# jiangzhengkai/mxdetection

Hardware: AMD Instinct MI355X
Metric: images/sec (whole node) Faster R-CNN R50-FPN 3x800x1333 (higher is better)
Workload: dtype bf16; 1 GPU; Faster R-CNN ResNet-50-FPN bf16 train step, batch 2/GPU, 3x800x1333 (padded 1344); global_batch=2, parallelism=dp1, frozen=stem+C2, frozen BN folded, optimizer=SGD momentum 0.9 wd 1e-4, launch=hipGraph replay, input=resident, wgrad_side_stream=True, rpn_branch_stream=True, grouped_wgrad=True, filter_prefetch_hints=True, params_trainable=41538304

## Files before the change

include/mxdet.h:

```cpp
#ifndef MXDET_H_
#define MXDET_H_

#include <stddef.h>
#include <stdint.h>

#ifdef __cplusplus
extern "C" {
#endif

#define MXDET_OK 0
#define MXDET_EINVAL (-1)
#define MXDET_ESHAPE (-2)
#define MXDET_EWORKSPACE (-3)
#define MXDET_EHIP (-4)
#define MXDET_ERCCL (-5)

#define MXDET_DTYPE_F32 0
#define MXDET_DTYPE_BF16 1

typedef void* mxdet_stream_t;

const char* mxdet_last_error(void);
const char* mxdet_version(void);

int mxdet_box_iou(const float* boxes_a, int64_t na, const float* boxes_b, int64_t nb, float* out,
                  mxdet_stream_t stream);

int mxdet_generate_anchors(const float* base_anchors, int32_t A, int32_t H, int32_t W, int32_t stride,
                           float* out, mxdet_stream_t stream);

size_t mxdet_nms_batched_workspace_bytes(int32_t B, int32_t n_max);
int mxdet_nms_batched(const float* boxes, const int32_t* counts, const uint8_t* invalid, int32_t B,
                      int32_t n_max, float thresh, int32_t max_keep, int32_t* keep_idx,
                      int32_t* num_keep, void* workspace, size_t workspace_bytes,
                      mxdet_stream_t stream);

size_t mxdet_detection_postprocess_workspace_bytes(int32_t N, int32_t rois_per_image, int32_t num_classes);
int mxdet_detection_postprocess(const void* cls_logits, const void* bbox_pred, int32_t dtype, int32_t ld_cls,
                                int32_t ld_reg, const float* rois, const int32_t* num_rois, const float* im_info,
                                int32_t N, int32_t rois_per_image, int32_t num_classes, const float* means,
                                const float* stds, float score_thresh, float nms_thresh, int32_t max_per_image,
                                float* dets, int32_t* num_dets, void* workspace, size_t workspace_bytes,
                                mxdet_stream_t stream);


typedef struct {
  int32_t num_levels;
  int32_t A;
  int32_t H[8], W[8], stride[8];
  const void* cls[8];
  const void* reg[8];
  int64_t cls_sn[8], cls_sy[8], cls_sx[8], cls_sa[8];
  int64_t reg_sn[8], reg_sy[8], reg_sx[8], reg_sc[8];
  int32_t dtype;
  int32_t classes;
  const float* base_anchors[8];
} mxdet_pyramid_t;

size_t mxdet_proposal_workspace_bytes(const mxdet_pyramid_t* p, int32_t N, int32_t pre_nms_top_n);
int mxdet_proposal(const mxdet_pyramid_t* p, int32_t N, const float* im_info ,
                   int32_t pre_nms_top_n, int32_t post_nms_top_n, float nms_thresh, float min_size,
                   float* rois, float* roi_scores, int32_t* roi_anchor, int32_t* num_rois,
                   void* workspace, size_t workspace_bytes, mxdet_stream_t stream);

size_t mxdet_anchor_target_workspace_bytes(int32_t N, int64_t A_total, int32_t G_max);
int mxdet_anchor_target(const float* anchors, int64_t A_total, const float* gt_boxes, int32_t N,
                        int32_t G_max, const float* im_info, float fg_thresh, float bg_thresh,
                        float allowed_border, int32_t batch_size, float fg_fraction, uint32_t seed,
                        uint32_t step, const uint32_t* step_dev, uint32_t image_offset, int32_t* labels,
                        int32_t* matched_gt,
                        float* bbox_targets, float* max_iou, void* workspace, size_t workspace_bytes,
                        mxdet_stream_t stream);

int mxdet_proposal_target(const float* rois, const int32_t* num_rois, int32_t rois_stride,
                          const float* gt_boxes, int32_t N, int32_t G_max, int32_t rois_per_image,
                          float fg_fraction, float fg_thresh, float bg_hi, float bg_lo,
                          int32_t num_classes, int32_t class_agnostic,
                          const float* means , const float* stds ,
                          uint32_t seed, uint32_t step, const uint32_t* step_dev,
                          uint32_t image_offset, float* out_rois, int32_t* labels,
                          float* bbox_targets, float* bbox_weights, int32_t* matched_gt,
                          int32_t* num_fg, mxdet_stream_t stream);

int mxdet_fpn_level_map(const float* rois, int64_t R, int32_t lvl_min, int32_t lvl_max,
                        int32_t* levels, mxdet_stream_t stream);
typedef struct {
  int32_t num_levels, lvl_min;
  int32_t H[8], W[8];
  float spatial_scale[8];
  void* feat[8];
} mxdet_feat_pyramid_t;
int mxdet_roi_align_fwd(const mxdet_feat_pyramid_t* f, int32_t N, int32_t C, const float* rois,
                        const int32_t* levels, int64_t R, int32_t PH, int32_t PW,
                        int32_t sampling_ratio, uint16_t* out, mxdet_stream_t stream);
int mxdet_roi_align_bwd(const mxdet_feat_pyramid_t* f, int32_t N, int32_t C, const float* rois,
                        const int32_t* levels, int64_t R, int32_t PH, int32_t PW,
                        int32_t sampling_ratio, const uint16_t* grad_out, mxdet_stream_t stream);
size_t mxdet_roi_align_bwd_gather_workspace_bytes(const mxdet_feat_pyramid_t* f, int32_t N, int64_t R);
int mxdet_roi_align_bwd_gather(const mxdet_feat_pyramid_t* f, int32_t N, int32_t C, const float* rois,
                               const int32_t* levels, int64_t R, int32_t PH, int32_t PW, int32_t sampling_ratio,
                               const uint16_t* grad_out, int32_t accumulate, void* workspace, size_t workspace_bytes,
                               mxdet_stream_t stream);
int mxdet_roi_align_bwd_gather_prepare(const mxdet_feat_pyramid_t* f, int32_t N, const float* rois,
                                       const int32_t* levels, int64_t R, int32_t PH, int32_t PW, int32_t sampling_ratio,
                                       void* workspace, size_t workspace_bytes, mxdet_stream_t stream);
int mxdet_roi_align_bwd_gather_prepared(const mxdet_feat_pyramid_t* f, int32_t N, int32_t C, const float* rois,
                                        const int32_t* levels, int64_t R, int32_t PH, int32_t PW, int32_t sampling_ratio,
                                        const uint16_t* grad_out, int32_t accumulate, void* workspace,
                                        size_t workspace_bytes, mxdet_stream_t stream);

typedef struct {
  mxdet_feat_pyramid_t pyr;
  int32_t N, C;
  int32_t PH, PW;
  int32_t sample_per_part;
  float trans_std;
  int32_t modulated;
  int32_t trans_stride, mask_stride;
  int32_t accumulate;
} mxdet_dpool_desc_t;
int mxdet_dpool_fwd(const mxdet_dpool_desc_t* d, const float* rois, const int32_t* levels, int64_t R,
                    const uint16_t* trans, const uint16_t* mask_logit, uint16_t* out, mxdet_stream_t stream);
int mxdet_dpool_bwd_trans(const mxdet_dpool_desc_t* d, const float* rois, const int32_t* levels, int64_t R,
                          const uint16_t* trans, const uint16_t* mask_logit, const uint16_t* dout, uint16_t* d_trans,
                          uint16_t* d_mask, mxdet_stream_t stream);
size_t mxdet_dpool_bwd_feat_workspace_bytes(const mxdet_dpool_desc_t* d, int64_t R);
int mxdet_dpool_bwd_feat(const mxdet_dpool_desc_t* d, const float* rois, const int32_t* levels, int64_t R,
                         const uint16_t* trans, const uint16_t* mask_logit, const uint16_t* dout, void* workspace,
                         size_t workspace_bytes, mxdet_stream_t stream);

int mxdet_smooth_l1_fwd(const float* pred, const float* target, const float* weight, int64_t n,
                        float sigma, float* out, mxdet_stream_t stream);
int mxdet_smooth_l1_bwd(const float* pred, const float* target, const float* weight,
                        const float* grad_out, int64_t n, float sigma, int32_t accumulate,
                        float* grad_pred, mxdet_stream_t stream);

size_t mxdet_loss_workspace_bytes(int64_t n);
int mxdet_focal_loss(const void* logits, int32_t dtype, const int32_t* labels, int64_t n, int32_t C,
                     float alpha, float gamma, float grad_scale, float* loss_out, void* grad_logits,
                     void* workspace, size_t workspace_bytes, mxdet_stream_t stream);

int mxdet_anchor_class_labels(const int32_t* labels, const int32_t* matched_gt, const float* gt_boxes, int32_t N,
                              int64_t A_total, int32_t G_max, int32_t* cls_labels, int32_t* num_fg,
                              mxdet_stream_t stream);
int32_t mxdet_retina_loss_num_partials(int32_t N, int32_t H, int32_t W, int32_t A);
int mxdet_retina_loss_level(const uint16_t* cls, const uint16_t* reg, int32_t N, int32_t H, int32_t W, int32_t A,
                            int32_t C, int32_t ld_cls, int32_t ld_reg, const int32_t* cls_labels,
                            const float* bbox_targets, int64_t A_total, int64_t level_offset, float alpha,
                            float gamma, float sigma, const int32_t* num_fg, float loss_scale, uint16_t* grad_cls,
                            uint16_t* grad_reg, float* partial, mxdet_stream_t stream);

int32_t mxdet_rpn_loss_num_partials(int32_t N, int32_t H, int32_t W);
int mxdet_rpn_loss_level(const uint16_t* head, int32_t N, int32_t H, int32_t W, int32_t A,
                         int32_t Cpad, const int32_t* labels, const float* bbox_targets,
                         int64_t A_total, int64_t level_offset, float sigma, float norm,
                         float loss_scale, uint16_t* grad_head, float* partial,
                         mxdet_stream_t stream);
int mxdet_loss_finalize(const float* partial, int32_t count, int32_t ncomp, float* out,
                        mxdet_stream_t stream);

int mxdet_rcnn_loss(const void* cls_logits, const void* bbox_pred, int32_t dtype, int32_t ld_cls,
                    int32_t ld_reg, const int32_t* labels, const float* bbox_targets,
                    const float* bbox_weights, int64_t R, int32_t num_classes, int32_t reg_dim,
                    float sigma, float norm, float loss_scale, float* loss_out, void* grad_cls,
                    void* grad_reg, void* workspace, size_t workspace_bytes, mxdet_stream_t stream);

int mxdet_mask_target(const float* rois, const int32_t* matched_gt, const int32_t* labels,
                      const uint8_t* gt_masks, int64_t R, int32_t G_max, int32_t H, int32_t W, int32_t S,
                      uint8_t* targets, int32_t* cls_out, mxdet_stream_t stream);
int mxdet_pixel_shuffle2(const uint16_t* x, int64_t R, int32_t H, int32_t W, int32_t C, int32_t inverse,
                         uint16_t* y, mxdet_stream_t stream);
int mxdet_pixel_shuffle2_inv_relu(const uint16_t* dy_up, const uint16_t* act, int64_t R, int32_t H, int32_t W, int32_t C,
                                  uint16_t* dx, mxdet_stream_t stream);
size_t mxdet_mask_loss_workspace_bytes(int64_t R, int32_t S);
int mxdet_mask_loss(const uint16_t* logits, const int32_t* cls, const uint8_t* targets, int64_t R, int32_t S,
                    int32_t Cpad, float loss_scale, float* loss_out, uint16_t* grad, void* workspace,
                    size_t workspace_bytes, mxdet_stream_t stream);
size_t mxdet_mask_paste_workspace_bytes(int64_t R, int32_t S);
int mxdet_mask_paste(const uint16_t* logits, const float* dets, int64_t R, int32_t S, int32_t Cpad, int32_t H, int32_t W,
                     float thresh, uint8_t* masks, void* workspace, size_t workspace_bytes, mxdet_stream_t stream);

typedef struct {
  int32_t N, H, W, Cin;
  int32_t Cout, KH, KW;
  int32_t stride, pad;
  int32_t Ho, Wo;
  int32_t relu;
  int32_t res_upsample;
  int32_t accumulate;
  const void* prefetch;
  int64_t prefetch_bytes;
  void* relu_bits;
} mxdet_conv_desc_t;

int mxdet_conv2d_fwd(const mxdet_conv_desc_t* d, const uint16_t* x, const uint16_t* w,
                     const float* bias, const uint16_t* residual, uint16_t* y,
                     mxdet_stream_t stream);
int mxdet_conv2d_fwd_chain(const mxdet_conv_desc_t* d, const uint16_t* x, const uint16_t* w, const float* bias,
                           const uint16_t* w2, const float* bias2, int32_t cout2, int32_t relu2,
                           const uint16_t* residual2, uint16_t* y2, const uint16_t* w3, const float* bias3,
                           int32_t cout3, int32_t relu3, uint16_t* y3, mxdet_stream_t stream);
size_t mxdet_conv2d_fwd_splitk_workspace_bytes(const mxdet_conv_desc_t* d, int32_t ksplit);
int mxdet_conv2d_fwd_splitk(const mxdet_conv_desc_t* d, const uint16_t* x, const uint16_t* w, const float* bias,
                            const uint16_t* residual, uint16_t* y, int32_t ksplit, void* workspace,
                            size_t workspace_bytes, mxdet_stream_t stream);
int mxdet_conv2d_dgrad(const mxdet_conv_desc_t* d, const uint16_t* dy, const uint16_t* wt,
                       const uint16_t* residual, const uint16_t* relu_mask, uint16_t* dx,
                       mxdet_stream_t stream);
size_t mxdet_conv2d_wgrad_workspace_bytes(const mxdet_conv_desc_t* d);
int mxdet_conv2d_wgrad(const mxdet_conv_desc_t* d, const uint16_t* x, const uint16_t* dy, float* dw,
                       float* db, void* workspace, size_t workspace_bytes, mxdet_stream_t stream);
typedef struct {
  mxdet_conv_desc_t desc;
  const void* src;
  const void* filt;
  const float* bias;
  const void* residual;
  const void* relu_mask;
  void* dst;
} mxdet_conv_item_t;
size_t mxdet_conv2d_grouped_table_bytes(int32_t n);
int mxdet_conv2d_grouped_plan(const mxdet_conv_item_t* items, int32_t n, int32_t kind, void* table_host,
                              size_t table_bytes, int32_t* cfg, int32_t* grid);
int mxdet_conv2d_grouped(const void* table_dev, int32_t n, int32_t kind, int32_t cfg, int32_t grid,
                         mxdet_stream_t stream);
typedef struct {
  mxdet_conv_desc_t desc;
  const void* x;
  const void* dy;
  float* dw;
  float* db;
} mxdet_wgrad_item_t;
size_t mxdet_conv2d_wgrad_grouped_table_bytes(int32_t n);
int mxdet_conv2d_wgrad_grouped_plan(const mxdet_wgrad_item_t* items, int32_t n, void* table_host, size_t table_bytes,
                                    size_t* workspace_bytes, int32_t* grid_wgrad, int32_t* grid_big,
                                    int32_t* grid_reduce);
int mxdet_conv2d_wgrad_grouped(const void* table_dev, int32_t n, int32_t grid_wgrad, int32_t grid_big,
                               int32_t grid_reduce, void* workspace, size_t workspace_bytes, size_t workspace_needed,
                               mxdet_stream_t stream);
int mxdet_conv2d_wgrad_grouped_parts(const void* table_dev, int32_t n, int32_t grid_wgrad, int32_t grid_big,
                                     int32_t grid_reduce, int32_t parts, void* workspace, size_t workspace_bytes,
                                     size_t workspace_needed, mxdet_stream_t stream);
int mxdet_filter_transpose(const uint16_t* w, int32_t Cout, int32_t KH, int32_t KW, int32_t Cin,
                           uint16_t* wt, mxdet_stream_t stream);

int mxdet_filter_transpose_batched(const void* descs_dev, int32_t ndesc, int32_t total_tiles,
                                   mxdet_stream_t stream);

typedef struct {
  int32_t N, H, W, C;
  int32_t Ho, Wo;
  int32_t KH, KW;
  int32_t stride, pad;
  int32_t groups;
  int32_t modulated;
  int32_t off_channels;
  int32_t accumulate;
} mxdet_deform_desc_t;
int mxdet_deform_im2col(const mxdet_deform_desc_t* d, const uint16_t* x, const uint16_t* off, uint16_t* col,
                        mxdet_stream_t stream);
int mxdet_deform_col2im_coord(const mxdet_deform_desc_t* d, const uint16_t* x, const uint16_t* off,
                              const uint16_t* dcol, uint16_t* doff, mxdet_stream_t stream);
size_t mxdet_deform_col2im_workspace_bytes(const mxdet_deform_desc_t* d);
int mxdet_deform_col2im(const mxdet_deform_desc_t* d, const uint16_t* off, const uint16_t* dcol, uint16_t* dx,
                        void* workspace, size_t workspace_bytes, mxdet_stream_t stream);

typedef struct {
  int32_t N, HW, C, G;
  float eps;
  int32_t relu;
  int32_t accumulate;
} mxdet_gn_desc_t;
size_t mxdet_group_norm_workspace_bytes(const mxdet_gn_desc_t* d, int32_t backward);
int mxdet_group_norm_fwd(const mxdet_gn_desc_t* d, const uint16_t* x, const float* gamma, const float* beta, uint16_t* y,
                         float* mean, float* rstd, void* workspace, size_t workspace_bytes, mxdet_stream_t stream);
int mxdet_group_norm_bwd(const mxdet_gn_desc_t* d, const uint16_t* x, const uint16_t* dy, const uint16_t* y,
                         const float* mean, const float* rstd, const float* gamma, const float* beta, uint16_t* dx,
                         float* dgamma, float* dbeta, void* workspace, size_t workspace_bytes, mxdet_stream_t stream);

int mxdet_stem_conv7x7(const void* image, int32_t dtype, int32_t N, int32_t H, int32_t W,
                       const uint16_t* w, const float* bias, uint16_t* y, mxdet_stream_t stream);
int mxdet_stem_conv7x7_pool(const void* image, int32_t dtype, int32_t N, int32_t H, int32_t W,
                            const uint16_t* w, const float* bias, uint16_t* y, mxdet_stream_t stream);
int mxdet_maxpool3x3s2(const uint16_t* x, int32_t N, int32_t H, int32_t W, int32_t C, uint16_t* y,
                       mxdet_stream_t stream);
int mxdet_subsample2(const uint16_t* x, int32_t N, int32_t H, int32_t W, int32_t C, uint16_t* y,
                     mxdet_stream_t stream);
int mxdet_subsample2_bwd(const uint16_t* dy, int32_t N, int32_t H, int32_t W, int32_t C,
                         int32_t accumulate, uint16_t* dx, mxdet_stream_t stream);
int mxdet_upsample2_bwd(const uint16_t* dfine, int32_t N, int32_t Hf, int32_t Wf, int32_t C,
                        int32_t accumulate, uint16_t* dcoarse, mxdet_stream_t stream);
size_t mxdet_retina_detect_workspace_bytes(const mxdet_pyramid_t* p, int32_t N, int32_t pre_nms_top_n);
int mxdet_retina_detect(const mxdet_pyramid_t* p, int32_t N, const float* im_info, int32_t pre_nms_top_n,
                        float score_thresh, float nms_thresh, int32_t max_per_image, float* dets, int32_t* num_dets,
                        void* workspace, size_t workspace_bytes, mxdet_stream_t stream);

typedef struct {
  const uint8_t* src;
  int32_t src_h, src_w;
  int32_t dst_h, dst_w;
  int32_t flip;
  int32_t pad_;
  double inv_scale;
} mxdet_image_desc_t;
#define MXDET_PREPROCESS_MAX_BATCH 64
int mxdet_image_preprocess(const mxdet_image_desc_t* images , int32_t N, int32_t Hp, int32_t Wp,
                           const float* mean3 , const float* std3 , int32_t swap_rb,
                           uint16_t* out, mxdet_stream_t stream);

int mxdet_polygon_masks(const float* verts, const int32_t* poly_start, const int32_t* inst_first, int32_t N,
                        int32_t G, int32_t H, int32_t W, uint8_t* masks, mxdet_stream_t stream);

int mxdet_add_bf16(const uint16_t* a, const uint16_t* b, int64_t n, uint16_t* out,
                   mxdet_stream_t stream);
int mxdet_relu_bwd_bf16(const uint16_t* dy, const uint16_t* y, int64_t n, uint16_t* dx,
                        mxdet_stream_t stream);
int mxdet_f32_to_bf16(const float* x, int64_t n, uint16_t* y, mxdet_stream_t stream);
int mxdet_f32_accum_to_bf16(const float* x, int64_t n, int32_t accumulate, uint16_t* y,
                            mxdet_stream_t stream);
int mxdet_nchw_to_nhwc_bf16(const void* x, int32_t dtype, int32_t N, int32_t C, int32_t H, int32_t W,
                            uint16_t* y, mxdet_stream_t stream);
int mxdet_nhwc_to_nchw_f32(const uint16_t* x, int32_t N, int32_t C, int32_t H, int32_t W, float* y,
                           mxdet_stream_t stream);

int mxdet_sgd_momentum_update(float* w, const float* grad, float* mom, uint16_t* w_bf16, int64_t n,
                              float lr, float momentum, float wd, float rescale,
                              mxdet_stream_t stream);
int mxdet_sgd_momentum_update_sched(float* w, const float* grad, float* mom, uint16_t* w_bf16, int64_t n,
                                    const float* lr_dev, float momentum, float wd, float rescale,
                                    mxdet_stream_t stream);

typedef struct mxdet_comm mxdet_comm_t;
#define MXDET_COMM_ID_BYTES 128
#define MXDET_COMM_MAX_INFLIGHT 64
int mxdet_comm_unique_id(uint8_t* id );
int mxdet_comm_create(const uint8_t* id, int32_t world, int32_t rank, mxdet_comm_t** comm_out);
int mxdet_comm_destroy(mxdet_comm_t* comm);
int mxdet_allreduce_bucket(mxdet_comm_t* comm, float* grad, int64_t count, mxdet_stream_t stream,
                           int32_t* ticket_out);
int mxdet_comm_wait(mxdet_comm_t* comm, int32_t ticket, mxdet_stream_t stream);
int mxdet_comm_broadcast(mxdet_comm_t* comm, void* buf, size_t bytes, int32_t root, mxdet_stream_t stream);

#ifdef __cplusplus
}
#endif
#endif
```

include/mxdet_debug.h:

```cpp
#ifndef MXDET_DEBUG_H_
#define MXDET_DEBUG_H_

#include <stdint.h>

#include "mxdet.h"

#ifdef __cplusplus
extern "C" {
#endif

int mxdet_debug_force_conv_cfg(int32_t cfg);
int mxdet_debug_force_wgrad_ksplit(int32_t ksplit);
int mxdet_debug_preprocess_direct(int32_t on);

#define MXDET_TUNE_T64 0
#define MXDET_TUNE_T128 1
#define MXDET_TUNE_PAR64 2
#define MXDET_TUNE_WG_TARGET 3
#define MXDET_TUNE_WG_MINSTEPS 4
#define MXDET_TUNE_WG_MAXSTEPS 5
#define MXDET_TUNE_T3_ENABLE 6
#define MXDET_TUNE_T3_TARGET 7
#define MXDET_TUNE_T3_MINSTEPS 8
#define MXDET_TUNE_T3_NS 9
#define MXDET_TUNE_TAIL 10
#define MXDET_TUNE_WG_NS 11
#define MXDET_TUNE_ROI_TABLE 12
#define MXDET_TUNE_ROI_ROWS 13
#define MXDET_TUNE_STATIC_TAPS 14
#define MXDET_TUNE_T128W 15
#define MXDET_TUNE_T3_MIX 16
#define MXDET_TUNE_SPLITK_TILE 17
#define MXDET_TUNE_T3_PER_ITEM 18
#define MXDET_TUNE_COUNT 19
int mxdet_debug_set_tuning(int32_t which, int64_t value);
int64_t mxdet_debug_get_tuning(int32_t which);


#define MXDET_ROUTE_CONV 1
#define MXDET_ROUTE_WGRAD 2
#define MXDET_ROUTE_CONV_GROUPED 3
#define MXDET_ROUTE_WGRAD_GROUPED 4
#define MXDET_ROUTE_WORDS 16
#define MXDET_ROUTE_MAX 4
int mxdet_debug_route_probe(int32_t on);
int mxdet_debug_route_read(int32_t* records, int32_t max_records);

#define MXDET_GN_ROUTE_RESIDENT 1
#define MXDET_GN_ROUTE_TILED 2
int mxdet_debug_group_norm_route(const mxdet_gn_desc_t* d);

#ifdef __cplusplus
}
#endif
#endif
```

mxdetection_amd/_lib.py:

```python
import ctypes as C
import os

_HERE = os.path.dirname(os.path.abspath(__file__))
LIB_PATH = os.environ.get("MXDET_LIB") or os.path.join(_HERE, "libmxdet_hip.so")

c_i32, c_i64, c_u32, c_f32, c_sz, c_vp = C.c_int32, C.c_int64, C.c_uint32, C.c_float, C.c_size_t, C.c_void_p


class PyramidT(C.Structure):
    _fields_ = [
        ("num_levels", c_i32), ("A", c_i32),
        ("H", c_i32 * 8), ("W", c_i32 * 8), ("stride", c_i32 * 8),
        ("cls", c_vp * 8), ("reg", c_vp * 8),
        ("cls_sn", c_i64 * 8), ("cls_sy", c_i64 * 8), ("cls_sx", c_i64 * 8), ("cls_sa", c_i64 * 8),
        ("reg_sn", c_i64 * 8), ("reg_sy", c_i64 * 8), ("reg_sx", c_i64 * 8), ("reg_sc", c_i64 * 8),
        ("dtype", c_i32), ("classes", c_i32),
        ("base_anchors", c_vp * 8),
    ]


class FeatPyramidT(C.Structure):
    _fields_ = [
        ("num_levels", c_i32), ("lvl_min", c_i32),
        ("H", c_i32 * 8), ("W", c_i32 * 8),
        ("spatial_scale", c_f32 * 8),
        ("feat", c_vp * 8),
    ]


class ImageDescT(C.Structure):
    _fields_ = [("src", C.c_void_p), ("src_h", C.c_int32), ("src_w", C.c_int32), ("dst_h", C.c_int32),
                ("dst_w", C.c_int32), ("flip", C.c_int32), ("pad_", C.c_int32), ("inv_scale", C.c_double)]


class WgradItemT(C.Structure):
    pass


class ConvItemT(C.Structure):
    pass


class ConvDescT(C.Structure):
    _fields_ = [
        ("N", c_i32), ("H", c_i32), ("W", c_i32), ("Cin", c_i32),
        ("Cout", c_i32), ("KH", c_i32), ("KW", c_i32),
        ("stride", c_i32), ("pad", c_i32),
        ("Ho", c_i32), ("Wo", c_i32),
        ("relu", c_i32), ("res_upsample", c_i32), ("accumulate", c_i32),
        ("prefetch", c_vp), ("prefetch_bytes", c_i64), ("relu_bits", c_vp),
    ]


class DeformDescT(C.Structure):
    _fields_ = [
        ("N", c_i32), ("H", c_i32), ("W", c_i32), ("C", c_i32),
        ("Ho", c_i32), ("Wo", c_i32), ("KH", c_i32), ("KW", c_i32),
        ("stride", c_i32), ("pad", c_i32), ("groups", c_i32), ("modulated", c_i32),
        ("off_channels", c_i32), ("accumulate", c_i32),
    ]


class DpoolDescT(C.Structure):
    _fields_ = [
        ("pyr", FeatPyramidT), ("N", c_i32), ("C", c_i32), ("PH", c_i32), ("PW", c_i32),
        ("sample_per_part", c_i32), ("trans_std", c_f32), ("modulated", c_i32),
        ("trans_stride", c_i32), ("mask_stride", c_i32), ("accumulate", c_i32),
    ]


class GnDescT(C.Structure):
    _fields_ = [("N", c_i32), ("HW", c_i32), ("C", c_i32), ("G", c_i32), ("eps", c_f32), ("relu", c_i32),
                ("accumulate", c_i32)]


WgradItemT._fields_ = [("desc", ConvDescT), ("x", c_vp), ("dy", c_vp), ("dw", c_vp), ("db", c_vp)]
ConvItemT._fields_ = [("desc", ConvDescT), ("src", c_vp), ("filt", c_vp), ("bias", c_vp), ("residual", c_vp),
                      ("relu_mask", c_vp), ("dst", c_vp)]

P = C.POINTER

SIGNATURES = {
    "mxdet_last_error": (C.c_char_p, []),
    "mxdet_version": (C.c_char_p, []),
    "mxdet_box_iou": (c_i32, [c_vp, c_i64, c_vp, c_i64, c_vp, c_vp]),
    "mxdet_generate_anchors": (c_i32, [c_vp, c_i32, c_i32, c_i32, c_i32, c_vp, c_vp]),
    "mxdet_nms_batched_workspace_bytes": (c_sz, [c_i32, c_i32]),
    "mxdet_nms_batched": (c_i32, [c_vp, c_vp, c_vp, c_i32, c_i32, c_f32, c_i32, c_vp, c_vp, c_vp, c_sz, c_vp]),
    "mxdet_pixel_shuffle2_inv_relu": (c_i32, [c_vp, c_vp, c_i64, c_i32, c_i32, c_i32, c_vp, c_vp]),
    "mxdet_mask_paste_workspace_bytes": (c_sz, [c_i64, c_i32]),
    "mxdet_mask_paste": (c_i32, [c_vp, c_vp, c_i64, c_i32, c_i32, c_i32, c_i32, c_f32, c_vp, c_vp, c_sz, c_vp]),
    "mxdet_retina_detect_workspace_bytes": (c_sz, [c_vp, c_i32, c_i32]),
    "mxdet_retina_detect": (c_i32, [c_vp, c_i32, c_vp, c_i32, c_f32, c_f32, c_i32, c_vp, c_vp, c_vp, c_sz, c_vp]),
    "mxdet_debug_preprocess_direct": (c_i32, [c_i32]),
    "mxdet_image_preprocess": (c_i32, [c_vp, c_i32, c_i32, c_i32, c_vp, c_vp, c_i32, c_vp, c_vp]),
    "mxdet_polygon_masks": (c_i32, [c_vp, c_vp, c_vp, c_i32, c_i32, c_i32, c_i32, c_vp, c_vp]),
    "mxdet_detection_postprocess_workspace_bytes": (c_sz, [c_i32, c_i32, c_i32]),
    "mxdet_detection_postprocess": (c_i32, [c_vp, c_vp, c_i32, c_i32, c_i32, c_vp, c_vp, c_vp, c_i32, c_i32, c_i32,
                                            P(c_f32), P(c_f32), c_f32, c_f32, c_i32, c_vp, c_vp, c_vp, c_sz, c_vp]),
    "mxdet_proposal_workspace_bytes": (c_sz, [P(PyramidT), c_i32, c_i32]),
    "mxdet_proposal": (c_i32, [P(PyramidT), c_i32, c_vp, c_i32, c_i32, c_f32, c_f32, c_vp, c_vp, c_vp, c_vp,
                               c_vp, c_sz, c_vp]),
    "mxdet_anchor_target_workspace_bytes": (c_sz, [c_i32, c_i64, c_i32]),
    "mxdet_anchor_target": (c_i32, [c_vp, c_i64, c_vp, c_i32, c_i32, c_vp, c_f32, c_f32, c_f32, c_i32, c_f32,
                                    c_u32, c_u32, c_vp, c_u32, c_vp, c_vp, c_vp, c_vp, c_vp, c_sz, c_vp]),
    "mxdet_proposal_target": (c_i32, [c_vp, c_vp, c_i32, c_vp, c_i32, c_i32, c_i32, c_f32, c_f32, c_f32, c_f32,
                                      c_i32, c_i32, P(c_f32), P(c_f32), c_u32, c_u32, c_vp, c_u32, c_vp, c_vp, c_vp,
                                      c_vp, c_vp, c_vp, c_vp]),
    "mxdet_fpn_level_map": (c_i32, [c_vp, c_i64, c_i32, c_i32, c_vp, c_vp]),
    "mxdet_roi_align_fwd": (c_i32, [P(FeatPyramidT), c_i32, c_i32, c_vp, c_vp, c_i64, c_i32, c_i32, c_i32, c_vp,
                                    c_vp]),
    "mxdet_roi_align_bwd": (c_i32, [P(FeatPyramidT), c_i32, c_i32, c_vp, c_vp, c_i64, c_i32, c_i32, c_i32, c_vp,
                                    c_vp]),
    "mxdet_roi_align_bwd_gather_workspace_bytes": (c_sz, [P(FeatPyramidT), c_i32, c_i64]),
    "mxdet_roi_align_bwd_gather": (c_i32, [P(FeatPyramidT), c_i32, c_i32, c_vp, c_vp, c_i64, c_i32, c_i32, c_i32, c_vp,
                                           c_i32, c_vp, c_sz, c_vp]),
    "mxdet_roi_align_bwd_gather_prepare": (c_i32, [P(FeatPyramidT), c_i32, c_vp, c_vp, c_i64, c_i32, c_i32, c_i32,
                                                   c_vp, c_sz, c_vp]),
    "mxdet_roi_align_bwd_gather_prepared": (c_i32, [P(FeatPyramidT), c_i32, c_i32, c_vp, c_vp, c_i64, c_i32, c_i32, c_i32,
                                                    c_vp, c_i32, c_vp, c_sz, c_vp]),
    "mxdet_smooth_l1_fwd": (c_i32, [c_vp, c_vp, c_vp, c_i64, c_f32, c_vp, c_vp]),
    "mxdet_smooth_l1_bwd": (c_i32, [c_vp, c_vp, c_vp, c_vp, c_i64, c_f32, c_i32, c_vp, c_vp]),
    "mxdet_loss_workspace_bytes": (c_sz, [c_i64]),
    "mxdet_focal_loss": (c_i32, [c_vp, c_i32, c_vp, c_i64, c_i32, c_f32, c_f32, c_f32, c_vp, c_vp, c_vp, c_sz,
                                 c_vp]),
    "mxdet_anchor_class_labels": (c_i32, [c_vp, c_vp, c_vp, c_i32, c_i64, c_i32, c_vp, c_vp, c_vp]),
    "mxdet_retina_loss_num_partials": (c_i32, [c_i32, c_i32, c_i32, c_i32]),
    "mxdet_retina_loss_level": (c_i32, [c_vp, c_vp, c_i32, c_i32, c_i32, c_i32, c_i32, c_i32, c_i32, c_vp, c_vp, c_i64,
                                        c_i64, c_f32, c_f32, c_f32, c_vp, c_f32, c_vp, c_vp, c_vp, c_vp]),
    "mxdet_rpn_loss_num_partials": (c_i32, [c_i32, c_i32, c_i32]),
    "mxdet_rpn_loss_level": (c_i32, [c_vp, c_i32, c_i32, c_i32, c_i32, c_i32, c_vp, c_vp, c_i64, c_i64, c_f32,
                                     c_f32, c_f32, c_vp, c_vp, c_vp]),
    "mxdet_loss_finalize": (c_i32, [c_vp, c_i32, c_i32, c_vp, c_vp]),
    "mxdet_rcnn_loss": (c_i32, [c_vp, c_vp, c_i32, c_i32, c_i32, c_vp, c_vp, c_vp, c_i64, c_i32, c_i32, c_f32,
                                c_f32, c_f32, c_vp, c_vp, c_vp, c_vp, c_sz, c_vp]),
    "mxdet_mask_target": (c_i32, [c_vp, c_vp, c_vp, c_vp, c_i64, c_i32, c_i32, c_i32, c_i32, c_vp, c_vp, c_vp]),
    "mxdet_pixel_shuffle2": (c_i32, [c_vp, c_i64, c_i32, c_i32, c_i32, c_i32, c_vp, c_vp]),
    "mxdet_mask_loss_workspace_bytes": (c_sz, [c_i64, c_i32]),
    "mxdet_mask_loss": (c_i32, [c_vp, c_vp, c_vp, c_i64, c_i32, c_i32, c_f32, c_vp, c_vp, c_vp, c_sz, c_vp]),
    "mxdet_conv2d_fwd": (c_i32, [P(ConvDescT), c_vp, c_vp, c_vp, c_vp, c_vp, c_vp]),
    "mxdet_conv2d_fwd_chain": (c_i32, [P(ConvDescT), c_vp, c_vp, c_vp, c_vp, c_vp, c_i32, c_i32, c_vp, c_vp, c_vp, c_vp, c_i32,
                                       c_i32, c_vp, c_vp]),
    "mxdet_conv2d_fwd_splitk_workspace_bytes": (c_sz, [P(ConvDescT), c_i32]),
    "mxdet_conv2d_fwd_splitk": (c_i32, [P(ConvDescT), c_vp, c_vp, c_vp, c_vp, c_vp, c_i32, c_vp, c_sz, c_vp]),
    "mxdet_conv2d_dgrad": (c_i32, [P(ConvDescT), c_vp, c_vp, c_vp, c_vp, c_vp, c_vp]),
    "mxdet_conv2d_wgrad_workspace_bytes": (c_sz, [P(ConvDescT)]),
    "mxdet_conv2d_wgrad": (c_i32, [P(ConvDescT), c_vp, c_vp, c_vp, c_vp, c_vp, c_sz, c_vp]),
    "mxdet_conv2d_grouped_table_bytes": (c_sz, [c_i32]),
    "mxdet_conv2d_grouped_plan": (c_i32, [P(ConvItemT), c_i32, c_i32, c_vp, c_sz, P(c_i32), P(c_i32)]),
    "mxdet_conv2d_grouped": (c_i32, [c_vp, c_i32, c_i32, c_i32, c_i32, c_vp]),
    "mxdet_conv2d_wgrad_grouped_table_bytes": (c_sz, [c_i32]),
    "mxdet_conv2d_wgrad_grouped_plan": (c_i32, [P(WgradItemT), c_i32, c_vp, c_sz, P(c_sz), P(c_i32), P(c_i32), P(c_i32)]),
    "mxdet_conv2d_wgrad_grouped": (c_i32, [c_vp, c_i32, c_i32, c_i32, c_i32, c_vp, c_sz, c_sz, c_vp]),
    "mxdet_conv2d_wgrad_grouped_parts": (c_i32, [c_vp, c_i32, c_i32, c_i32, c_i32, c_i32, c_vp, c_sz, c_sz, c_vp]),
    "mxdet_debug_force_conv_cfg": (c_i32, [c_i32]),
    "mxdet_debug_force_wgrad_ksplit": (c_i32, [c_i32]),
    "mxdet_filter_transpose": (c_i32, [c_vp, c_i32, c_i32, c_i32, c_i32, c_vp, c_vp]),
    "mxdet_filter_transpose_batched": (c_i32, [c_vp, c_i32, c_i32, c_vp]),
    "mxdet_deform_im2col": (c_i32, [P(DeformDescT), c_vp, c_vp, c_vp, c_vp]),
    "mxdet_deform_col2im_coord": (c_i32, [P(DeformDescT), c_vp, c_vp, c_vp, c_vp, c_vp]),
    "mxdet_deform_col2im_workspace_bytes": (c_sz, [P(DeformDescT)]),
    "mxdet_deform_col2im": (c_i32, [P(DeformDescT), c_vp, c_vp, c_vp, c_vp, c_sz, c_vp]),
    "mxdet_dpool_fwd": (c_i32, [P(DpoolDescT), c_vp, c_vp, c_i64, c_vp, c_vp, c_vp, c_vp]),
    "mxdet_dpool_bwd_trans": (c_i32, [P(DpoolDescT), c_vp, c_vp, c_i64, c_vp, c_vp, c_vp, c_vp, c_vp, c_vp]),
    "mxdet_dpool_bwd_feat_workspace_bytes": (c_sz, [P(DpoolDescT), c_i64]),
    "mxdet_dpool_bwd_feat": (c_i32, [P(DpoolDescT), c_vp, c_vp, c_i64, c_vp, c_vp, c_vp, c_vp, c_sz, c_vp]),
    "mxdet_group_norm_workspace_bytes": (c_sz, [P(GnDescT), c_i32]),
    "mxdet_group_norm_fwd": (c_i32, [P(GnDescT), c_vp, c_vp, c_vp, c_vp, c_vp, c_vp, c_vp, c_sz, c_vp]),
    "mxdet_group_norm_bwd": (c_i32, [P(GnDescT), c_vp, c_vp, c_vp, c_vp, c_vp, c_vp, c_vp, c_vp, c_vp, c_vp, c_vp, c_sz,
                                     c_vp]),
    "mxdet_debug_group_norm_route": (c_i32, [P(GnDescT)]),
    "mxdet_stem_conv7x7": (c_i32, [c_vp, c_i32, c_i32, c_i32, c_i32, c_vp, c_vp, c_vp, c_vp]),
    "mxdet_stem_conv7x7_pool": (c_i32, [c_vp, c_i32, c_i32, c_i32, c_i32, c_vp, c_vp, c_vp, c_vp]),
    "mxdet_maxpool3x3s2": (c_i32, [c_vp, c_i32, c_i32, c_i32, c_i32, c_vp, c_vp]),
    "mxdet_subsample2": (c_i32, [c_vp, c_i32, c_i32, c_i32, c_i32, c_vp, c_vp]),
    "mxdet_subsample2_bwd": (c_i32, [c_vp, c_i32, c_i32, c_i32, c_i32, c_i32, c_vp, c_vp]),
    "mxdet_upsample2_bwd": (c_i32, [c_vp, c_i32, c_i32, c_i32, c_i32, c_i32, c_vp, c_vp]),
    "mxdet_add_bf16": (c_i32, [c_vp, c_vp, c_i64, c_vp, c_vp]),
    "mxdet_relu_bwd_bf16": (c_i32, [c_vp, c_vp, c_i64, c_vp, c_vp]),
    "mxdet_f32_to_bf16": (c_i32, [c_vp, c_i64, c_vp, c_vp]),
    "mxdet_f32_accum_to_bf16": (c_i32, [c_vp, c_i64, c_i32, c_vp, c_vp]),
    "mxdet_nchw_to_nhwc_bf16": (c_i32, [c_vp, c_i32, c_i32, c_i32, c_i32, c_i32, c_vp, c_vp]),
    "mxdet_nhwc_to_nchw_f32": (c_i32, [c_vp, c_i32, c_i32, c_i32, c_i32, c_vp, c_vp]),
    "mxdet_sgd_momentum_update": (c_i32, [c_vp, c_vp, c_vp, c_vp, c_i64, c_f32, c_f32, c_f32, c_f32, c_vp]),
    "mxdet_sgd_momentum_update_sched": (c_i32, [c_vp, c_vp, c_vp, c_vp, c_i64, c_vp, c_f32, c_f32, c_f32, c_vp]),
    "mxdet_comm_unique_id": (c_i32, [c_vp]),
    "mxdet_comm_create": (c_i32, [c_vp, c_i32, c_i32, P(c_vp)]),
    "mxdet_comm_destroy": (c_i32, [c_vp]),
    "mxdet_allreduce_bucket": (c_i32, [c_vp, c_vp, c_i64, c_vp, P(c_i32)]),
    "mxdet_comm_wait": (c_i32, [c_vp, c_i32, c_vp]),
    "mxdet_comm_broadcast": (c_i32, [c_vp, c_vp, c_sz, c_i32, c_vp]),
    "mxdet_debug_set_tuning": (c_i32, [c_i32, c_i64]),
    "mxdet_debug_get_tuning": (c_i64, [c_i32]),
    "mxdet_debug_route_probe": (c_i32, [c_i32]),
    "mxdet_debug_route_read": (c_i32, [P(c_i32), c_i32]),
}

DEBUG_SYMBOLS = ("mxdet_debug_force_conv_cfg", "mxdet_debug_force_wgrad_ksplit", "mxdet_debug_preprocess_direct",
                 "mxdet_debug_set_tuning", "mxdet_debug_get_tuning", "mxdet_debug_route_probe", "mxdet_debug_route_read",
                 "mxdet_debug_group_norm_route")
TUNING_KEYS = {"T64": 0, "T128": 1, "PAR64": 2, "WG_TARGET": 3, "WG_MINSTEPS": 4, "WG_MAXSTEPS": 5, "T3_ENABLE": 6,
               "T3_TARGET": 7, "T3_MINSTEPS": 8, "T3_NS": 9, "TAIL": 10, "WG_NS": 11, "ROI_TABLE": 12, "ROI_ROWS": 13, "STATIC_TAPS": 14,
               "T128W": 15, "T3_MIX": 16, "SPLITK_TILE": 17, "T3_PER_ITEM": 18}

_lib = None


class MxdetError(RuntimeError):
    pass


def load():
    global _lib
    if _lib is not None:
        return _lib
    if not os.path.exists(LIB_PATH):
        raise MxdetError(
            "libmxdet_hip.so not found at %s -- build it with `python -m mxdetection_amd.build` "
            "(there is no CPU fallback)" % LIB_PATH)
    import torch
    lib = C.CDLL(LIB_PATH)
    for name, (res, args) in SIGNATURES.items():
        fn = getattr(lib, name, None)
        if fn is None:
            continue
        fn.restype = res
        fn.argtypes = args
    _lib = lib
    for key, idx in TUNING_KEYS.items():
        v = os.environ.get("MXDET_TUNE_" + key)
        if v:
            lib.mxdet_debug_set_tuning(idx, int(v))
    return lib


def check(rc, what=""):
    if rc != 0:
        msg = load().mxdet_last_error().decode("utf-8", "replace")
        raise MxdetError("%s failed (%d): %s" % (what or "mxdet call", rc, msg))


def ptr(t):
    return None if t is None else C.c_void_p(t.data_ptr())


def stream_ptr():
    import torch
    return C.c_void_p(torch.cuda.current_stream().cuda_stream)
```

mxdetection_amd/csrc/conv.hip:

```cpp
#include <stdlib.h>

#include "common.h"

namespace mxdet {

typedef __attribute__((ext_vector_type(8))) __bf16 bf16x8_t;
typedef __attribute__((ext_vector_type(4))) float f32x4_t;

struct ConvP {
  const uint16_t* x;
  const uint16_t* w;
  const float* bias;
  const uint16_t* res;
  const uint16_t* mask;
  uint16_t* y;
  int N, Hs, Ws, C;
  int Hd, Wd, Ncols;
  int KH, KW, stride, pad;
  int relu, res_up;
  int M;
  int tiles_m, tiles_n;
  int par_tile0[5];
  int par_hc[2], par_wc[2];
  int par_h0[2], par_w0[2];
  int m_begin;
  int ksplit;
  float* partial;
  const void* pf;
  long long pf_bytes;
  unsigned char* bits_out;
  const unsigned char* bits_in;
  int force_cfg;
  const uint16_t* chain_w;
  const float* chain_bias;
  const uint16_t* chain_res;
  uint16_t* chain_y;
  int chain_relu;
  const uint16_t* chain3_w;
  const float* chain3_bias;
  uint16_t* chain3_y;
  int chain3_relu;
};

__device__ __forceinline__ int lds_off(int row, int chunk) {
  return row * 64 + ((chunk ^ ((row >> 1) & 7)) << 3);
}

typedef const __attribute__((address_space(1))) void* gptr_t;
typedef __attribute__((address_space(3))) void* lptr_t;

#ifdef MXDET_CONV_STAMP
__device__ unsigned long long g_conv_stamp[2][8];
#define MXDET_CS(k) do { if (cs_on) cs[k] = __builtin_amdgcn_s_memtime(); } while (0)
#else
#define MXDET_CS(k) do { } while (0)
#endif

template <int BM, int BN, int WM, int WN, int NS, bool DGRAD, bool PAR = false, int TAPS = 0, int CHAIN = 0>
__device__ __forceinline__ void conv_igemm_tile(const ConvP& p, int bid, const int nwg) {
  constexpr int NW = WM * WN, NTHR = 64 * NW;
  constexpr int WTM = BM / WM, WTN = BN / WN;
  constexpr int MT = WTM / 16, NT = WTN / 16;
  constexpr int NBUF = NS;
  constexpr int RPI = 8;
  constexpr int GA = BM / RPI / NW, GB = BN / RPI / NW;
  constexpr int STAGE = (BM + BN) * 64;
  static_assert(BM % (RPI * NW) == 0 && BN % (RPI * NW) == 0, "rows must split evenly over the waves");
  static_assert(MT % 2 == 0, "epilogue stages two m-tiles at a time");
  static_assert(NS >= 2 && (NS - 2) * (GA + GB) <= 63, "vmcnt is a 6-bit counter");
  static_assert(TAPS == 0 || ((TAPS == 1 || TAPS == 9) && !PAR), "static taps: 1x1 or 3x3");
  constexpr int EP_STRIDE = WTN + 4;
  constexpr int EP_BYTES = NW * 32 * EP_STRIDE * 4;
  constexpr int MAIN_BYTES = NBUF * STAGE * 2;
  static_assert(CHAIN == 0 || (TAPS == 9 && !DGRAD && WN == 1 && BN == 64 && CHAIN % (8 * NW) == 0),
                "chain: forward 3x3 whose waves own all 64 mid channels of their rows");
  constexpr int CHAIN_OFF = MAIN_BYTES > EP_BYTES ? MAIN_BYTES : EP_BYTES;
  constexpr int SMEM_BYTES = CHAIN_OFF + CHAIN * 128;
  __shared__ __attribute__((aligned(1024))) unsigned char smem_raw[SMEM_BYTES];
  uint16_t* smem = (uint16_t*)smem_raw;

  const int tid = threadIdx.x, lane = tid & 63;
  const int wid = __builtin_amdgcn_readfirstlane(tid >> 6);
  const int wm = wid / WN, wn = wid % WN;
#ifdef MXDET_CONV_STAMP
  const bool cs_on = (blockIdx.x == 0 || blockIdx.x == 300) && wid == 0;
  unsigned long long cs[8] = {0, 0, 0, 0, 0, 0, 0, 0};
#endif
  MXDET_CS(0);

  const int pf_bid = bid, pf_nwg = nwg;
  int ks = 0, sl_begin = 0, sl_end = p.C >> 6;
  int nwg_ = nwg;
  if constexpr (TAPS == 1) {
    if (p.ksplit > 1) {
      const int tiles = p.tiles_m * p.tiles_n;
      ks = bid / tiles;
      bid -= ks * tiles;
      nwg_ = tiles;
      const int per = ((p.C >> 6) + p.ksplit - 1) / p.ksplit;
      sl_begin = ks * per;
      sl_end = sl_begin + per < sl_end ? sl_begin + per : sl_end;
      sl_end = sl_end < sl_begin ? sl_begin : sl_end;
    }
  }
  if constexpr (!PAR) {
    const int nwg = nwg_;
    int q = nwg >> 3, r = nwg & 7, xcd = bid & 7, idx = bid >> 3;
    bid = (xcd < r ? xcd * (q + 1) : r * (q + 1) + (xcd - r) * q) + idx;
  }
  const int tile_m = bid / p.tiles_n, tile_n = bid - tile_m * p.tiles_n;
  int m0 = p.m_begin + tile_m * BM;
  const int n0 = tile_n * BN;
  int par_ph = 0, par_pw = 0, par_rows = 0, par_hc = 1, par_wc = 1, nkh = p.KH, nkw = p.KW;
  if constexpr (PAR) {
    int c = 0;
    while (c < 3 && tile_m >= p.par_tile0[c + 1]) ++c;
    par_ph = c >> 1; par_pw = c & 1;
    par_hc = p.par_hc[par_ph]; par_wc = p.par_wc[par_pw];
    par_rows = p.N * par_hc * par_wc;
    m0 = (tile_m - p.par_tile0[c]) * BM;
    nkh = (p.KH - par_ph + 1) >> 1; nkw = (p.KW - par_pw + 1) >> 1;
    nkh = nkh < 0 ? 0 : nkh; nkw = nkw < 0 ? 0 : nkw;
  }

  const int lrow = lane >> 3, lslot = lane & 7;
  constexpr int SWZ = 7;
  const __amdgpu_buffer_rsrc_t rsrc_x = make_rsrc(p.x, 2u * (unsigned)(p.N * p.Hs * p.Ws) * (unsigned)p.C);
  const __amdgpu_buffer_rsrc_t rsrc_w = make_rsrc(p.w, 2u * (unsigned)p.Ncols * (unsigned)(p.KH * p.KW * p.C));
  const int ntaps = p.KH * p.KW;
  const int hw_d = p.Hd * p.Wd;
  const bool smallm = p.M < (1 << 24);
  const float rcp_hw = 1.0f / (float)hw_d, rcp_w = 1.0f / (float)p.Wd;
  const int Ktot = ntaps * p.C;
  const int KT = PAR ? (nkh * nkw * p.C) >> 6 : Ktot >> 6;
  int wrow[GB];
#pragma unroll
  for (int i = 0; i < GB; ++i) {
    int rb = (wid * GB + i) * RPI + lrow;
    int n = n0 + rb;
    n = n < p.Ncols ? n : p.Ncols - 1;
    wrow[i] = n * Ktot + ((lslot ^ ((rb >> 1) & SWZ)) << 3);
  }
  auto issue_b = [&](int buf, int tap, int c0, bool live) {
    const int so_b = live ? 2 * (tap * p.C + c0) : 0;
    unsigned char* sbase = smem_raw + (size_t)buf * (STAGE * 2);
#pragma unroll
    for (int i = 0; i < GB; ++i)
#if !defined(MXDET_ABL_NOLOAD) && !defined(MXDET_ABL_NOBLOAD)
      __builtin_amdgcn_raw_ptr_buffer_load_lds(rsrc_w, (lptr_t)(sbase + BM * 128 + (wid * GB + i) * 1024), 16,
                                               (int)(2u * (unsigned)wrow[i]), so_b, 0, 0);
#else
      asm volatile("" ::"v"(wrow[i]), "s"(so_b));
#endif
  };
  if constexpr (TAPS > 0) {
#pragma unroll
    for (int s0 = 0; s0 < NS - 1; ++s0)
      issue_b(s0, s0 % TAPS, (sl_begin + s0 / TAPS) * 64, s0 < (sl_end - sl_begin) * TAPS);
  }
  if constexpr (CHAIN > 0) {
    const __amdgpu_buffer_rsrc_t rsrc_c = make_rsrc(p.chain_w, 2u * (unsigned)CHAIN * 64u);
#pragma unroll
    for (int i = 0; i < CHAIN / 8 / NW; ++i) {
      const int r = (wid * (CHAIN / 8 / NW) + i) * 8 + lrow;
      const unsigned vo = 2u * (unsigned)(r * 64 + ((lslot ^ ((r >> 1) & 7)) << 3));
      __builtin_amdgcn_raw_ptr_buffer_load_lds(rsrc_c, (lptr_t)(smem_raw + CHAIN_OFF + (wid * (CHAIN / 8 / NW) + i) * 1024), 16,
                                               (int)vo, 0, 0, 0);
    }
  }
  int a_off[GA];
  unsigned a_mask[GA];
#pragma unroll
  for (int i = 0; i < GA; ++i) {
    int ra = (wid * GA + i) * RPI + lrow;
    int m = m0 + ra;
    int coff = (lslot ^ ((ra >> 1) & SWZ)) << 3;
    unsigned mask = 0;
    int off = 0;
    if constexpr (PAR) {
      if (m < par_rows) {
        int img = m / (par_hc * par_wc);
        int rem = m - img * (par_hc * par_wc);
        int ih = rem / par_wc, iw = rem - ih * par_wc;
        int hd = p.par_h0[par_ph] + 2 * ih, wd = p.par_w0[par_pw] + 2 * iw;
        int hs0 = (hd + p.pad - par_ph) >> 1, ws0 = (wd + p.pad - par_pw) >> 1;
        off = ((img * p.Hs + hs0) * p.Ws + ws0) * p.C + coff;
        for (int a = 0; a < nkh; ++a)
          for (int b = 0; b < nkw; ++b) {
            int hs = hs0 - a, ws = ws0 - b;
            if (hs >= 0 && ws >= 0 && hs < p.Hs && ws < p.Ws) mask |= 1u << (a * nkw + b);
          }
      }
    } else if (ntaps == 1 && p.stride == 1 && p.pad == 0) {
      if (m < p.M) { off = m * p.C + coff; mask = 1u; }
    } else
    if (m < p.M) {
      int img, hd, wd, rem;
      if (smallm) {
        img = fast_divmod(m, hw_d, rcp_hw, &rem);
        hd = fast_divmod(rem, p.Wd, rcp_w, &wd);
      } else {
        img = m / hw_d; rem = m - img * hw_d;
        hd = rem / p.Wd; wd = rem - hd * p.Wd;
      }
      int h0, w0;
      if (DGRAD) {
        if (p.stride == 1) { h0 = hd + p.pad; w0 = wd + p.pad; }
        else { h0 = (hd + p.pad) / p.stride; w0 = (wd + p.pad) / p.stride; }
      } else { h0 = hd * p.stride - p.pad; w0 = wd * p.stride - p.pad; }
      off = ((img * p.Hs + h0) * p.Ws + w0) * p.C + coff;
      if (DGRAD && p.stride != 1) {
        for (int kh = 0; kh < p.KH; ++kh)
          for (int kw = 0; kw < p.KW; ++kw) {
            int th = hd + p.pad - kh, tw = wd + p.pad - kw;
            int hs = th / p.stride, ws = tw / p.stride;
            bool ok = th >= 0 && tw >= 0 && th == hs * p.stride && tw == ws * p.stride && hs < p.Hs && ws < p.Ws;
            if (ok) mask |= 1u << (kh * p.KW + kw);
          }
      } else if (TAPS == 9) {
        const unsigned rlo = (DGRAD ? h0 < p.Hs : h0 >= 0) ? 1u : 0u, rhi = (DGRAD ? h0 - 2 >= 0 : h0 + 2 < p.Hs) ? 4u : 0u;
        const unsigned clo = (DGRAD ? w0 < p.Ws : w0 >= 0) ? 1u : 0u, chi = (DGRAD ? w0 - 2 >= 0 : w0 + 2 < p.Ws) ? 4u : 0u;
        const unsigned rowm = rlo | 2u | rhi, colm = clo | 2u | chi;
        mask = ((rowm & 1u) ? colm : 0u) | (colm << 3) | ((rowm & 4u) ? colm << 6 : 0u);
      } else {
        unsigned rowm = 0, colm = 0;
        for (int kh = 0; kh < p.KH; ++kh) {
          const int hs = DGRAD ? h0 - kh : h0 + kh;
          if (hs >= 0 && hs < p.Hs) rowm |= 1u << kh;
        }
        for (int kw = 0; kw < p.KW; ++kw) {
          const int ws = DGRAD ? w0 - kw : w0 + kw;
          if (ws >= 0 && ws < p.Ws) colm |= 1u << kw;
        }
        for (int kh = 0; kh < p.KH; ++kh)
          if ((rowm >> kh) & 1u) mask |= colm << (kh * p.KW);
      }
    }
    a_off[i] = off;
    a_mask[i] = mask;
  }

  auto issue_at = [&](int buf, int kh, int kw, int c0, bool live) {
    unsigned char* sbase = smem_raw + (size_t)buf * (STAGE * 2);
    const int tap = live ? kh * p.KW + kw : 31;
    const int delta = DGRAD ? c0 - (kh * p.Ws + kw) * p.C : c0 + (kh * p.Ws + kw) * p.C;
    const int koff = live ? (kh * p.KW + kw) * p.C + c0 : 0;
#pragma unroll
    for (int i = 0; i < GA; ++i) {
      const unsigned vo = ((a_mask[i] >> tap) & 1u) ? 2u * (unsigned)(a_off[i] + delta) : kDmaOob;
      __builtin_amdgcn_raw_ptr_buffer_load_lds(rsrc_x, (lptr_t)(sbase + (wid * GA + i) * 1024), 16, (int)vo, 0, 0, 0);
    }
#pragma unroll
    for (int i = 0; i < GB; ++i) {
      const unsigned wo = 2u * (unsigned)(wrow[i] + koff);
      __builtin_amdgcn_raw_ptr_buffer_load_lds(rsrc_w, (lptr_t)(sbase + BM * 128 + (wid * GB + i) * 1024), 16, (int)wo, 0, 0, 0);
    }
  };
  int ld_kt = 0, ld_kh = 0, ld_kw = 0, ld_c0 = 0;
  auto issue_stage = [&](int buf) {
    unsigned char* sbase = smem_raw + (size_t)buf * (STAGE * 2);
    const bool live = ld_kt < KT;
    int tap, delta, koff;
    if constexpr (PAR) {
      tap = live ? ld_kh * nkw + ld_kw : 31;
      delta = ld_c0 - (ld_kh * p.Ws + ld_kw) * p.C;
      koff = live ? ((par_ph + 2 * ld_kh) * p.KW + (par_pw + 2 * ld_kw)) * p.C + ld_c0 : 0;
    } else {
      tap = live ? ld_kh * p.KW + ld_kw : 31;
      if (DGRAD) delta = ld_c0 - ((ld_kh / p.stride) * p.Ws + (ld_kw / p.stride)) * p.C;
      else delta = ld_c0 + (ld_kh * p.Ws + ld_kw) * p.C;
      koff = live ? (ld_kh * p.KW + ld_kw) * p.C + ld_c0 : 0;
    }
#pragma unroll
    for (int i = 0; i < GA; ++i) {
      unsigned vo = ((a_mask[i] >> tap) & 1u) ? 2u * (unsigned)(a_off[i] + delta) : kDmaOob;
#ifdef MXDET_ABL_ZEROSRC
      vo = kDmaOob;
#endif
#ifndef MXDET_ABL_NOLOAD
      __builtin_amdgcn_raw_ptr_buffer_load_lds(rsrc_x, (lptr_t)(sbase + (wid * GA + i) * 1024), 16, (int)vo, 0, 0, 0);
#else
      asm volatile("" ::"v"(vo));
#endif
    }
#pragma unroll
    for (int i = 0; i < GB; ++i) {
      unsigned wo = 2u * (unsigned)(wrow[i] + koff);
#ifdef MXDET_ABL_ZEROSRC
      wo = kDmaOob;
#endif
#ifndef MXDET_ABL_NOLOAD
      __builtin_amdgcn_raw_ptr_buffer_load_lds(rsrc_w, (lptr_t)(sbase + BM * 128 + (wid * GB + i) * 1024), 16, (int)wo, 0, 0, 0);
#else
      asm volatile("" ::"v"(wo));
#endif
    }
    ++ld_kt;
    if (++ld_kw == nkw) {
      ld_kw = 0;
      if (++ld_kh == nkh) { ld_kh = 0; ld_c0 += 64; }
    }
  };

  f32x4_t acc[MT][NT];
#pragma unroll
  for (int i = 0; i < MT; ++i)
#pragma unroll
    for (int j = 0; j < NT; ++j) acc[i][j] = (f32x4_t){0.f, 0.f, 0.f, 0.f};
  MXDET_CS(1);

  const int frow = lane & 15, fq = lane >> 4;
  if constexpr (TAPS > 0) {
  constexpr int TKW = TAPS == 9 ? 3 : 1;
  constexpr int SL = (NS % TAPS == 0 || TAPS % NS == 0) ? (TAPS % NS == 0 ? 1 : NS) : NS;
  static_assert((SL * TAPS) % NS == 0, "the ring position must repeat with the unrolled block");
  const int bias_el = (p.pad * p.Ws + p.pad) * p.C;
  const int rebase = DGRAD ? ((p.KH - 1) * p.Ws + (p.KW - 1)) * p.C : 0;
  const __amdgpu_buffer_rsrc_t rsrc_xs =
      make_rsrc(p.x - bias_el, 2u * (unsigned)(p.N * p.Hs * p.Ws) * (unsigned)p.C + 2u * (unsigned)bias_el);
  unsigned voa[GA];
#pragma unroll
  for (int i = 0; i < GA; ++i) {
    voa[i] = 2u * (unsigned)(a_off[i] - rebase + bias_el);
    if (TAPS == 1) voa[i] = (a_mask[i] & 1u) ? voa[i] : kDmaOob;
  }
  auto issue_a = [&](int buf, int tap, int c0, bool live) {
    const int kh = tap / TKW, kw = tap % TKW;
    const int disp = DGRAD ? ((p.KH - 1 - kh) * p.Ws + (p.KW - 1 - kw)) * p.C : (kh * p.Ws + kw) * p.C;
    const int so_a = live ? 2 * (disp + c0) : 0;
    unsigned char* sbase = smem_raw + (size_t)buf * (STAGE * 2);
#pragma unroll
    for (int i = 0; i < GA; ++i) {
      unsigned vo = voa[i];
      if (TAPS != 1) vo = ((a_mask[i] >> tap) & 1u) ? vo : kDmaOob;
      if (!live) vo = kDmaOob;
#ifndef MXDET_ABL_NOLOAD
      __builtin_amdgcn_raw_ptr_buffer_load_lds(rsrc_xs, (lptr_t)(sbase + (wid * GA + i) * 1024), 16, (int)vo, so_a, 0, 0);
#else
      asm volatile("" ::"v"(vo), "s"(so_a));
#endif
    }
  };
  const uint16_t* fa0 = smem + lds_off(wm * WTM + frow, fq);
  const uint16_t* fa1 = smem + lds_off(wm * WTM + frow, 4 + fq);
  const uint16_t* fb0 = smem + BM * 64 + lds_off(wn * WTN + frow, fq);
  const uint16_t* fb1 = smem + BM * 64 + lds_off(wn * WTN + frow, 4 + fq);
  const int nslices = sl_end;
#pragma unroll
  for (int s0 = 0; s0 < NS - 1; ++s0)
    issue_a(s0, s0 % TAPS, (sl_begin + s0 / TAPS) * 64, s0 < (sl_end - sl_begin) * TAPS);
  asm volatile("s_waitcnt vmcnt(%0)" ::"n"((NS - 2) * GA) : "memory");
#ifdef MXDET_ABL_NOBFRAG
  bf16x8_t bf0[NT], bf1[NT];
#pragma unroll
  for (int j = 0; j < NT; ++j) { bf0[j] = *(const bf16x8_t*)(fb0 + j * 1024); bf1[j] = *(const bf16x8_t*)(fb1 + j * 1024); }
#endif
#ifdef MXDET_ABL_NOKLOOP
  for (int cs = sl_begin; cs < sl_begin; cs += SL) {
#else
  for (int cs = sl_begin; cs < nslices; cs += SL) {
#endif
#pragma unroll
    for (int sl = 0; sl < SL; ++sl) {
      if (SL > 1 && cs + sl >= nslices) break;
#pragma unroll
      for (int tp = 0; tp < TAPS; ++tp) {
        const int step = sl * TAPS + tp;
        const int cur = step % NS, nxt = (step + NS - 1) % NS;
        asm volatile("s_waitcnt vmcnt(%0)" ::"n"((NS - 2) * (GA + GB)) : "memory");
        __builtin_amdgcn_s_barrier();
        asm volatile("" ::: "memory");
#ifdef MXDET_ABL_NOBFRAG
        bf16x8_t af0[MT], af1[MT];
#else
        bf16x8_t af0[MT], bf0[NT], af1[MT], bf1[NT];
#endif
#pragma unroll
        for (int i = 0; i < MT; ++i) af0[i] = *(const bf16x8_t*)(fa0 + cur * STAGE + i * 1024);
#ifndef MXDET_ABL_NOBFRAG
#pragma unroll
        for (int j = 0; j < NT; ++j) bf0[j] = *(const bf16x8_t*)(fb0 + cur * STAGE + j * 1024);
#endif
#pragma unroll
        for (int i = 0; i < MT; ++i) af1[i] = *(const bf16x8_t*)(fa1 + cur * STAGE + i * 1024);
#ifndef MXDET_ABL_NOBFRAG
#pragma unroll
        for (int j = 0; j < NT; ++j) bf1[j] = *(const bf16x8_t*)(fb1 + cur * STAGE + j * 1024);
#endif
        __builtin_amdgcn_sched_barrier(0);
        {
          const int ahead = tp + NS - 1;
          const int atap = ahead % TAPS, aslice = ahead / TAPS;
          issue_a(nxt, atap, (cs + sl + aslice) * 64, cs + sl + aslice < nslices);
          issue_b(nxt, atap, (cs + sl + aslice) * 64, cs + sl + aslice < nslices);
        }
        __builtin_amdgcn_sched_barrier(0);
        __builtin_amdgcn_s_setprio(1);
#ifndef MXDET_ABL_NOMFMA
#pragma unroll
        for (int i = 0; i < MT; ++i)
#pragma unroll
          for (int j = 0; j < NT; ++j)
            acc[i][j] = __builtin_amdgcn_mfma_f32_16x16x32_bf16(af0[i], bf0[j], acc[i][j], 0, 0, 0);
#pragma unroll
        for (int i = 0; i < MT; ++i)
#pragma unroll
          for (int j = 0; j < NT; ++j)
            acc[i][j] = __builtin_amdgcn_mfma_f32_16x16x32_bf16(af1[i], bf1[j], acc[i][j], 0, 0, 0);
#else
#pragma unroll
        for (int i = 0; i < MT; ++i) { asm volatile("" ::"v"(af0[i])); asm volatile("" ::"v"(af1[i])); }
#pragma unroll
        for (int j = 0; j < NT; ++j) { asm volatile("" ::"v"(bf0[j])); asm volatile("" ::"v"(bf1[j])); }
#endif
        __builtin_amdgcn_sched_barrier(0);
        __builtin_amdgcn_s_setprio(0);
      }
    }
  }
  } else {
#pragma unroll
  for (int s0 = 0; s0 < NS - 1; ++s0) issue_stage(s0);

  int cur = 0, nxt = NS - 1;
  for (int kt = 0; kt < KT; ++kt) {
    asm volatile("s_waitcnt vmcnt(%0)" ::"n"((NS - 2) * (GA + GB)) : "memory");
    __builtin_amdgcn_s_barrier();
    asm volatile("" ::: "memory");
#ifdef MXDET_CONV_STAMP
    if (kt == 0) MXDET_CS(2);
#endif
    const uint16_t* sa = smem + cur * STAGE;
    const uint16_t* sb = sa + BM * 64;
    bf16x8_t af0[MT], bf0[NT], af1[MT], bf1[NT];
#pragma unroll
    for (int i = 0; i < MT; ++i) af0[i] = *(const bf16x8_t*)(sa + lds_off(wm * WTM + i * 16 + frow, fq));
#pragma unroll
    for (int j = 0; j < NT; ++j) bf0[j] = *(const bf16x8_t*)(sb + lds_off(wn * WTN + j * 16 + frow, fq));
    issue_stage(nxt);
    __builtin_amdgcn_s_setprio(1);
    __builtin_amdgcn_sched_barrier(0);
#pragma unroll
    for (int i = 0; i < MT; ++i) af1[i] = *(const bf16x8_t*)(sa + lds_off(wm * WTM + i * 16 + frow, 4 + fq));
#pragma unroll
    for (int j = 0; j < NT; ++j) bf1[j] = *(const bf16x8_t*)(sb + lds_off(wn * WTN + j * 16 + frow, 4 + fq));
#ifndef MXDET_ABL_NOMFMA
#pragma unroll
    for (int i = 0; i < MT; ++i)
#pragma unroll
      for (int j = 0; j < NT; ++j)
        acc[i][j] = __builtin_amdgcn_mfma_f32_16x16x32_bf16(af0[i], bf0[j], acc[i][j], 0, 0, 0);
#pragma unroll
    for (int g = 0; g < MT + NT; ++g) {
      __builtin_amdgcn_sched_group_barrier(0x008, (MT * NT) / (MT + NT), 0);
      __builtin_amdgcn_sched_group_barrier(0x100, 1, 0);
    }
#pragma unroll
    for (int i = 0; i < MT; ++i)
#pragma unroll
      for (int j = 0; j < NT; ++j)
        acc[i][j] = __builtin_amdgcn_mfma_f32_16x16x32_bf16(af1[i], bf1[j], acc[i][j], 0, 0, 0);
#else
#pragma unroll
    for (int i = 0; i < MT; ++i) { asm volatile("" ::"v"(af0[i])); asm volatile("" ::"v"(af1[i])); }
#pragma unroll
    for (int j = 0; j < NT; ++j) { asm volatile("" ::"v"(bf0[j])); asm volatile("" ::"v"(bf1[j])); }
#endif
    __builtin_amdgcn_sched_barrier(0);
    __builtin_amdgcn_s_setprio(0);
    cur = (cur + 1 == NS) ? 0 : cur + 1;
    nxt = (nxt + 1 == NS) ? 0 : nxt + 1;
  }
  }
  MXDET_CS(3);
  asm volatile("s_waitcnt vmcnt(0)" ::: "memory");
  __syncthreads();
  MXDET_CS(4);

  uint4 pfv[4] = {make_uint4(0u, 0u, 0u, 0u), make_uint4(0u, 0u, 0u, 0u), make_uint4(0u, 0u, 0u, 0u), make_uint4(0u, 0u, 0u, 0u)};
  if (p.pf != nullptr) {
    const long long pf_stride = (long long)pf_nwg * NTHR * 16;
    long long off = ((long long)pf_bid * NTHR + tid) * 16;
#pragma unroll
    for (int k = 0; k < 4; ++k, off += pf_stride)
      if (off + 16 <= p.pf_bytes) pfv[k] = *(const uint4*)((const char*)p.pf + off);
  }

  float* ep = (float*)smem_raw + wid * 32 * EP_STRIDE;
  constexpr int LPR = WTN / 8;
  constexpr int RPP = 64 / LPR;
  constexpr int PASSES = 32 / RPP;
  const int rl = lane / LPR, cg = lane - rl * LPR;
  bf16x8_t af2[CHAIN > 0 ? MT : 1][2];
  if constexpr (CHAIN > 0) {
#pragma unroll
    for (int i = 0; i < MT; ++i)
#pragma unroll
      for (int j = 0; j < NT; ++j)
#pragma unroll
        for (int r = 0; r < 4; ++r)
          ep[(i * 16 + fq * 4 + r) * EP_STRIDE + j * 16 + frow] = acc[i][j][r];
#pragma unroll
    for (int hf = 0; hf < 2; ++hf) {
      float4 c0 = make_float4(0.f, 0.f, 0.f, 0.f), c1 = c0;
      if (p.bias) {
        c0 = *(const float4*)(p.bias + hf * 32 + fq * 8);
        c1 = *(const float4*)(p.bias + hf * 32 + fq * 8 + 4);
      }
#pragma unroll
      for (int i = 0; i < MT; ++i) {
        const float4 v0 = *(const float4*)(ep + (i * 16 + frow) * EP_STRIDE + hf * 32 + fq * 8);
        const float4 v1 = *(const float4*)(ep + (i * 16 + frow) * EP_STRIDE + hf * 32 + fq * 8 + 4);
        float v[8] = {v0.x + c0.x, v0.y + c0.y, v0.z + c0.z, v0.w + c0.w, v1.x + c1.x, v1.y + c1.y, v1.z + c1.z, v1.w + c1.w};
        if (p.relu) {
#pragma unroll
          for (int k = 0; k < 8; ++k) v[k] = v[k] > 0.0f ? v[k] : 0.0f;
        }
        uint4 o;
        o.x = pack_bf16x2(v[0], v[1]);
        o.y = pack_bf16x2(v[2], v[3]);
        o.z = pack_bf16x2(v[4], v[5]);
        o.w = pack_bf16x2(v[6], v[7]);
        af2[i][hf] = __builtin_bit_cast(bf16x8_t, o);
      }
    }
  }
  static_assert(CHAIN == 0 || MT == 2, "chain: one epilogue half covers the wave's rows");
  constexpr int NCH = CHAIN > 0 ? CHAIN / BN : 1;
  const bool c3 = CHAIN > 0 && p.chain3_w != nullptr;
  f32x4_t acc3[CHAIN > 0 ? MT : 1][CHAIN > 0 ? NT : 1];
  if constexpr (CHAIN > 0) {
#pragma unroll
    for (int i = 0; i < MT; ++i)
#pragma unroll
      for (int j = 0; j < NT; ++j) acc3[i][j] = f32x4_t{0.f, 0.f, 0.f, 0.f};
  }
#pragma unroll 1
  for (int chunk = 0; chunk < (CHAIN > 0 ? NCH + (c3 ? 1 : 0) : 1); ++chunk) {
  const bool last3 = CHAIN > 0 && chunk == NCH;
  const int e_ncols = CHAIN > 0 ? (last3 ? BN : CHAIN) : p.Ncols;
  const float* const e_bias = CHAIN > 0 ? (last3 ? p.chain3_bias : p.chain_bias) : p.bias;
  const uint16_t* const e_res = CHAIN > 0 ? (last3 ? nullptr : p.chain_res) : p.res;
  uint16_t* const e_y = CHAIN > 0 ? (last3 ? p.chain3_y : p.chain_y) : p.y;
  const int e_relu = CHAIN > 0 ? (last3 ? p.chain3_relu : p.chain_relu) : p.relu;
  const int n0c = CHAIN > 0 ? (last3 ? 0 : chunk * BN) : n0;
  if constexpr (CHAIN > 0) {
    if (last3) {
#pragma unroll
      for (int i = 0; i < MT; ++i)
#pragma unroll
        for (int j = 0; j < NT; ++j) acc[i][j] = acc3[i][j];
    }
  }
  bf16x8_t b3[2][CHAIN > 0 ? NT : 1];
  if constexpr (CHAIN > 0) {
    if (c3 && !last3) {
#pragma unroll
      for (int hf = 0; hf < 2; ++hf)
#pragma unroll
        for (int j = 0; j < NT; ++j)
          b3[hf][j] = *(const bf16x8_t*)(p.chain3_w + (size_t)(j * 16 + frow) * CHAIN + chunk * BN + hf * 32 + fq * 8);
    }
  }
  if (CHAIN > 0 && !last3) {
    const uint16_t* wl = (const uint16_t*)(smem_raw + CHAIN_OFF);
#pragma unroll
    for (int i = 0; i < MT; ++i)
#pragma unroll
      for (int j = 0; j < NT; ++j) acc[i][j] = f32x4_t{0.f, 0.f, 0.f, 0.f};
#pragma unroll
    for (int hf = 0; hf < 2; ++hf) {
      bf16x8_t bw[NT];
#pragma unroll
      for (int j = 0; j < NT; ++j) bw[j] = *(const bf16x8_t*)(wl + lds_off(n0c + j * 16 + frow, hf * 4 + fq));
#pragma unroll
      for (int i = 0; i < MT; ++i)
#pragma unroll
        for (int j = 0; j < NT; ++j)
          acc[i][j] = __builtin_amdgcn_mfma_f32_16x16x32_bf16(af2[i][hf], bw[j], acc[i][j], 0, 0, 0);
    }
  }
  const int col = n0c + wn * WTN + cg * 8;
  const bool colok = col < e_ncols;
  float4 b0 = make_float4(0.f, 0.f, 0.f, 0.f), b1 = b0;
  if (e_bias) {
    const int cb = colok ? col : 0;
    b0 = *(const float4*)(e_bias + cb);
    b1 = *(const float4*)(e_bias + cb + 4);
  }
#pragma unroll
  for (int h = 0; h < MT / 2; ++h) {
    size_t pixs[PASSES];
    bool oks[PASSES];
    uint4 rres[PASSES], rmsk[PASSES];
#pragma unroll
    for (int ps = 0; ps < PASSES; ++ps) {
      const int row = ps * RPP + rl;
      const int m = m0 + wm * WTM + h * 32 + row;
      bool rowok = m < p.M;
      size_t pix = (size_t)m;
      if constexpr (PAR) {
        rowok = m < par_rows;
        int img = m / (par_hc * par_wc);
        int rem = m - img * (par_hc * par_wc);
        int ih = rem / par_wc, iw = rem - ih * par_wc;
        pix = (size_t)(img * p.Hd + p.par_h0[par_ph] + 2 * ih) * p.Wd + (p.par_w0[par_pw] + 2 * iw);
      }
      oks[ps] = rowok && colok;
      pixs[ps] = oks[ps] ? pix : 0;
    }
    if (e_res) {
#pragma unroll
      for (int ps = 0; ps < PASSES; ++ps) {
        size_t ri = pixs[ps] * e_ncols + (oks[ps] ? col : 0);
        if (CHAIN == 0 && p.res_up) {
          const int m = (int)pixs[ps];
          int img = m / (p.Hd * p.Wd);
          int rem = m - img * (p.Hd * p.Wd);
          int hd = rem / p.Wd, wd = rem - hd * p.Wd;
          int Hc = (p.Hd + 1) >> 1, Wc = (p.Wd + 1) >> 1;
          ri = ((size_t)(img * Hc + (hd >> 1)) * Wc + (wd >> 1)) * e_ncols + (oks[ps] ? col : 0);
        }
        rres[ps] = *(const uint4*)(e_res + ri);
      }
    }
    if (CHAIN == 0 && p.mask) {
#pragma unroll
      for (int ps = 0; ps < PASSES; ++ps)
        rmsk[ps] = *(const uint4*)(p.mask + pixs[ps] * e_ncols + (oks[ps] ? col : 0));
    }
    unsigned rbits[PASSES];
    if (CHAIN == 0 && p.bits_in) {
#pragma unroll
      for (int ps = 0; ps < PASSES; ++ps)
        rbits[ps] = p.bits_in[(pixs[ps] * e_ncols + (oks[ps] ? col : 0)) >> 3];
    }
#pragma unroll
    for (int t = 0; t < 2; ++t)
#pragma unroll
      for (int j = 0; j < NT; ++j)
#pragma unroll
        for (int r = 0; r < 4; ++r)
          ep[(t * 16 + fq * 4 + r) * EP_STRIDE + j * 16 + frow] = acc[2 * h + t][j][r];
#pragma unroll
    for (int ps = 0; ps < PASSES; ++ps) {
      const int row = ps * RPP + rl;
      float4 v0 = *(const float4*)(ep + row * EP_STRIDE + cg * 8);
      float4 v1 = *(const float4*)(ep + row * EP_STRIDE + cg * 8 + 4);
      if constexpr (TAPS == 1) {
        if (p.ksplit > 1) {
          if (oks[ps]) {
            float* dst = p.partial + ((size_t)ks * p.M + pixs[ps]) * e_ncols + col;
            *(float4*)dst = v0;
            *(float4*)(dst + 4) = v1;
          }
          continue;
        }
      }
      float v[8] = {v0.x + b0.x, v0.y + b0.y, v0.z + b0.z, v0.w + b0.w, v1.x + b1.x, v1.y + b1.y, v1.z + b1.z, v1.w + b1.w};
      if (e_res) {
        const uint4 rv = rres[ps];
        v[0] += __uint_as_float(rv.x << 16); v[1] += __uint_as_float(rv.x & 0xffff0000u);
        v[2] += __uint_as_float(rv.y << 16); v[3] += __uint_as_float(rv.y & 0xffff0000u);
        v[4] += __uint_as_float(rv.z << 16); v[5] += __uint_as_float(rv.z & 0xffff0000u);
        v[6] += __uint_as_float(rv.w << 16); v[7] += __uint_as_float(rv.w & 0xffff0000u);
      }
      if (CHAIN == 0 && p.mask) {
        const unsigned mm[4] = {rmsk[ps].x, rmsk[ps].y, rmsk[ps].z, rmsk[ps].w};
#pragma unroll
        for (int k = 0; k < 4; ++k) {
          unsigned lo = mm[k] & 0xffffu, hi = mm[k] >> 16;
          if (!(lo != 0u && lo < 0x8000u)) v[2 * k] = 0.0f;
          if (!(hi != 0u && hi < 0x8000u)) v[2 * k + 1] = 0.0f;
        }
      }
      if (CHAIN == 0 && p.bits_in) {
        const unsigned mb = rbits[ps];
#pragma unroll
        for (int k = 0; k < 8; ++k)
          if (!((mb >> k) & 1u)) v[k] = 0.0f;
      }
      if (e_relu && (CHAIN > 0 || (!p.mask && !p.bits_in))) {
#pragma unroll
        for (int k = 0; k < 8; ++k) v[k] = v[k] > 0.0f ? v[k] : 0.0f;
      }
      uint4 o;
      o.x = pack_bf16x2(v[0], v[1]);
      o.y = pack_bf16x2(v[2], v[3]);
      o.z = pack_bf16x2(v[4], v[5]);
      o.w = pack_bf16x2(v[6], v[7]);
      if (oks[ps]) *(uint4*)(e_y + pixs[ps] * e_ncols + col) = o;
      if constexpr (CHAIN > 0) {
        if (c3 && !last3) *(uint4*)((unsigned char*)ep + row * (EP_STRIDE * 4) + ((cg ^ (row & 7)) << 4)) = o;
      }
      if (CHAIN == 0 && p.bits_out && oks[ps]) {
        const unsigned w4[4] = {o.x, o.y, o.z, o.w};
        unsigned mb = 0;
#pragma unroll
        for (int k = 0; k < 4; ++k) {
          const unsigned lo = w4[k] & 0xffffu, hi = w4[k] >> 16;
          mb |= ((lo != 0u && lo < 0x8000u) ? 1u : 0u) << (2 * k);
          mb |= ((hi != 0u && hi < 0x8000u) ? 1u : 0u) << (2 * k + 1);
        }
        p.bits_out[(pixs[ps] * e_ncols + col) >> 3] = (unsigned char)mb;
      }
    }
  }
  if constexpr (CHAIN > 0) {
    if (c3 && !last3) {
#pragma unroll
      for (int hf = 0; hf < 2; ++hf) {
        bf16x8_t a3[MT];
#pragma unroll
        for (int i = 0; i < MT; ++i)
          a3[i] = *(const bf16x8_t*)((const unsigned char*)ep + (i * 16 + frow) * (EP_STRIDE * 4) +
                                     (((hf * 4 + fq) ^ ((i * 16 + frow) & 7)) << 4));
#pragma unroll
        for (int i = 0; i < MT; ++i)
#pragma unroll
          for (int j = 0; j < NT; ++j)
            acc3[i][j] = __builtin_amdgcn_mfma_f32_16x16x32_bf16(a3[i], b3[hf][j], acc3[i][j], 0, 0, 0);
      }
    }
  }
  }
  if (p.pf != nullptr) asm volatile("" ::"v"(pfv[0].x), "v"(pfv[1].x), "v"(pfv[2].x), "v"(pfv[3].x));
#ifdef MXDET_CONV_STAMP
  if (cs_on) {
    asm volatile("s_waitcnt vmcnt(0)" ::: "memory");
    cs[5] = __builtin_amdgcn_s_memtime();
    if (lane == 0)
      for (int k = 0; k < 6; ++k) g_conv_stamp[blockIdx.x == 0 ? 0 : 1][k] = cs[k];
  }
#endif
}

template <int BM, int BN, int WM, int WN, int NS, bool DGRAD, bool PAR = false, int TAPS = 0, int CHAIN = 0>
__global__ void __launch_bounds__(64 * WM * WN)
conv_igemm_kernel(ConvP p) {
  conv_igemm_tile<BM, BN, WM, WN, NS, DGRAD, PAR, TAPS, CHAIN>(p, (int)blockIdx.x, (int)gridDim.x);
}

struct ConvG {
  ConvP p;
  int block0, nblocks;
};

template <int BM, int BN, int WM, int WN, int NS, bool DGRAD, int TAPS = 0>
__global__ void __launch_bounds__(64 * WM * WN)
conv_igemm_grouped_kernel(const ConvG* __restrict__ table, int n) {
  int lo = 0, hi = n - 1;
  const int bid = (int)blockIdx.x;
  while (lo < hi) {
    int mid = (lo + hi + 1) >> 1;
    if (table[mid].block0 <= bid) lo = mid; else hi = mid - 1;
  }
  const int b = bid - table[lo].block0;
  const int nb = table[lo].nblocks;
  if (b >= nb) return;
  const ConvP p = table[lo].p;
  conv_igemm_tile<BM, BN, WM, WN, NS, DGRAD, false, TAPS>(p, b, nb);
}

static thread_local int g_force_cfg = 0;

static int thr_t64() { return (int)tuning(MXDET_TUNE_T64); }
static int thr_t128() { return (int)tuning(MXDET_TUNE_T128); }
static int thr_par64() { return (int)tuning(MXDET_TUNE_PAR64); }

template <int BM, int BN, int WM, int WN, int NS, bool DGRAD, bool PAR = false, int TAPS = 0, int CHAIN = 0>
static int launch_cfg(ConvP& p, hipStream_t s) {
  if (PAR) {
    int t = 0;
    for (int c = 0; c < 4; ++c) {
      p.par_tile0[c] = t;
      t += ceil_div(p.N * p.par_hc[c >> 1] * p.par_wc[c & 1], BM);
    }
    p.par_tile0[4] = t;
    p.tiles_m = t;
  }
  if (p.tiles_m <= 0) p.tiles_m = ceil_div(p.M - p.m_begin, BM);
  p.tiles_n = ceil_div(p.Ncols, BN);
  long long nwg = (long long)p.tiles_m * p.tiles_n;
  if (TAPS == 1 && p.ksplit > 1) nwg *= p.ksplit;
  if (route_probe_on()) {
    const int32_t rec[kRouteWords] = {MXDET_ROUTE_CONV, BM, BN, WM, WN, NS, DGRAD, PAR, TAPS, CHAIN, p.tiles_m, p.tiles_n,
                                      p.m_begin, p.ksplit, (int32_t)nwg, 0};
    route_record(rec);
    return MXDET_OK;
  }
  hipLaunchKernelGGL((conv_igemm_kernel<BM, BN, WM, WN, NS, DGRAD, PAR, TAPS, CHAIN>), dim3((unsigned)nwg),
                     dim3(64 * WM * WN), 0, s, p);
  return check_launch("conv2d");
}

template <bool DGRAD>
static int launch(ConvP& p, hipStream_t s) {
  const int force = g_force_cfg;
  const long long t128 = (long long)ceil_div(p.M, 128) * ceil_div(p.Ncols, 128);
  const long long t64 = (long long)ceil_div(p.M, 64) * ceil_div(p.Ncols, 128);
  const int K = p.KH * p.KW * p.C;
#define MXDET_FORCE_ST(BM, BN, WM, WN, NS)                                                  \
  (p.KH * p.KW == 1 ? launch_cfg<BM, BN, WM, WN, NS, DGRAD, false, 1>(p, s) : launch_cfg<BM, BN, WM, WN, NS, DGRAD, false, 9>(p, s))
  switch (force) {
    case 3: return launch_cfg<128, 128, 2, 2, 4, DGRAD>(p, s);
    case 5: return launch_cfg<64, 64, 2, 2, 3, DGRAD>(p, s);
    case 6: return launch_cfg<64, 128, 2, 2, 2, DGRAD>(p, s);
    case 7: return launch_cfg<128, 128, 2, 2, 2, DGRAD>(p, s);
    case 8: return launch_cfg<128, 64, 4, 1, 2, DGRAD>(p, s);
    case 15: return launch_cfg<256, 256, 2, 4, 2, DGRAD>(p, s);
    case 40: return MXDET_FORCE_ST(64, 64, 2, 2, 3);
    case 41: return MXDET_FORCE_ST(64, 128, 2, 2, 2);
    case 45: return MXDET_FORCE_ST(128, 128, 2, 2, 2);
    case 46: return MXDET_FORCE_ST(128, 64, 4, 1, 2);
    case 49: return MXDET_FORCE_ST(128, 128, 2, 4, 2);
    default: break;
  }
#undef MXDET_FORCE_ST
  const int taps = p.KH * p.KW;
  const int st = ((p.stride != 1 && (DGRAD || taps == 1)) || tuning(MXDET_TUNE_STATIC_TAPS) == 0) ? 0
                 : (taps == 1 && p.pad == 0) ? 1 : (p.KH == 3 && p.KW == 3 && p.pad == 1) ? 9 : 0;
#define MXDET_LAUNCH_ST(BM, BN, WM, WN, NS)                                                        \
  (st == 1 ? launch_cfg<BM, BN, WM, WN, NS, DGRAD, false, 1>(p, s)                                 \
           : st == 9 ? launch_cfg<BM, BN, WM, WN, NS, DGRAD, false, 9>(p, s)                       \
                     : launch_cfg<BM, BN, WM, WN, NS, DGRAD>(p, s))
  if constexpr (DGRAD) {
    if (p.stride == 2 && force == 0) {
      for (int par = 0; par < 2; ++par) {
        int h0 = ((par - p.pad) % 2 + 2) % 2, w0 = h0;
        p.par_h0[par] = h0; p.par_w0[par] = w0;
        p.par_hc[par] = p.Hd > h0 ? (p.Hd - h0 + 1) / 2 : 0;
        p.par_wc[par] = p.Wd > w0 ? (p.Wd - w0 + 1) / 2 : 0;
      }
      if (p.Ncols <= 64) return launch_cfg<128, 64, 4, 1, 2, true, true>(p, s);
      if (t64 >= thr_par64()) return launch_cfg<64, 128, 2, 2, 2, true, true>(p, s);
      return launch_cfg<64, 64, 2, 2, 3, true, true>(p, s);
    }
  }
  if (p.Ncols <= 64) return MXDET_LAUNCH_ST(128, 64, 4, 1, 2);
  if (t128 >= thr_t128() && K > 256) {
    const int tn = ceil_div(p.Ncols, 256);
    const long long full = (long long)(p.M / 256) * tn;
    const long long rounds = full / 256;
    if (rounds >= 1 && p.Ncols % 256 == 0) {
      ConvP big = p;
      big.tiles_m = (int)(rounds * 256 / tn);
      int rc = launch_cfg<256, 256, 2, 4, 2, DGRAD>(big, s);
      if (rc) return rc;
      p.m_begin = big.tiles_m * 256;
      if (p.m_begin >= p.M) return rc;
    }
    switch ((int)tuning(MXDET_TUNE_TAIL)) {
      case 1: return MXDET_LAUNCH_ST(64, 128, 2, 2, 2);
      case 2: return MXDET_LAUNCH_ST(64, 64, 2, 2, 3);
      default: return MXDET_LAUNCH_ST(128, 128, 2, 2, 2);
    }
  }
  {
    const long long t256 = (long long)(p.M / 256) * (p.Ncols / 256);
    if (p.M % 256 == 0 && p.Ncols % 256 == 0 && t256 >= 160 && t256 <= 256 && K >= 1024 && p.m_begin == 0)
      return launch_cfg<256, 256, 2, 4, 2, DGRAD>(p, s);
  }
  if (st != 0 && p.Ncols >= 128 && t128 >= tuning(MXDET_TUNE_T128W)) return MXDET_LAUNCH_ST(128, 128, 2, 4, 2);
  if (t64 >= thr_t64()) return MXDET_LAUNCH_ST(64, 128, 2, 2, 2);
  return MXDET_LAUNCH_ST(64, 64, 2, 2, 3);
#undef MXDET_LAUNCH_ST
}

static int validate(const mxdet_conv_desc_t* d, const char* who) {
  MXDET_REQUIRE(d != nullptr, MXDET_EINVAL, "%s: null descriptor", who);
  MXDET_REQUIRE(d->N > 0 && d->H > 0 && d->W > 0 && d->Cin > 0 && d->Cout > 0 && d->KH > 0 && d->KW > 0 &&
                    d->stride > 0 && d->pad >= 0,
                MXDET_ESHAPE, "%s: non-positive dimension", who);
  MXDET_REQUIRE(d->KH * d->KW <= 25, MXDET_ESHAPE, "%s: at most 25 filter taps (use the stem kernel for 7x7)", who);
  MXDET_REQUIRE(d->Ho == (d->H + 2 * d->pad - d->KH) / d->stride + 1 &&
                    d->Wo == (d->W + 2 * d->pad - d->KW) / d->stride + 1,
                MXDET_ESHAPE, "%s: Ho/Wo do not match the convolution arithmetic", who);
  MXDET_REQUIRE((long long)d->N * d->H * d->W * d->Cin < (1ll << 31) &&
                    (long long)d->N * d->Ho * d->Wo * d->Cout < (1ll << 31),
                MXDET_ESHAPE, "%s: tensor exceeds 2^31 elements", who);
  return MXDET_OK;
}

}

using namespace mxdet;

#ifdef MXDET_CONV_STAMP
extern "C" int mxdet_debug_read_conv_stamps(unsigned long long* out ) {
  return hipMemcpyFromSymbol(out, HIP_SYMBOL(g_conv_stamp), sizeof(unsigned long long) * 16) == hipSuccess ? 0 : -4;
}
#endif

extern "C" int mxdet_debug_force_conv_cfg(int32_t cfg) {
  g_force_cfg = cfg;
  return MXDET_OK;
}

extern "C" int mxdet_conv2d_fwd(const mxdet_conv_desc_t* d, const uint16_t* x, const uint16_t* w,
                                const float* bias, const uint16_t* residual, uint16_t* y,
                                mxdet_stream_t stream) {
  clear_error();
  int rc = validate(d, "conv2d_fwd");
  if (rc) return rc;
  MXDET_REQUIRE(d->Cin % 64 == 0, MXDET_ESHAPE, "conv2d_fwd: Cin %d must be a multiple of 64", d->Cin);
  MXDET_REQUIRE(d->Cout % 8 == 0, MXDET_ESHAPE, "conv2d_fwd: Cout %d must be a multiple of 8", d->Cout);
  MXDET_REQUIRE(x && w && y, MXDET_EINVAL, "conv2d_fwd: null pointer");
  ConvP p;
  memset(&p, 0, sizeof(p));
  p.x = x; p.w = w; p.bias = bias; p.res = residual; p.mask = nullptr; p.y = y;
  p.N = d->N; p.Hs = d->H; p.Ws = d->W; p.C = d->Cin;
  p.Hd = d->Ho; p.Wd = d->Wo; p.Ncols = d->Cout;
  p.KH = d->KH; p.KW = d->KW; p.stride = d->stride; p.pad = d->pad;
  p.relu = d->relu; p.res_up = d->res_upsample;
  p.M = d->N * d->Ho * d->Wo;
  p.pf = d->prefetch; p.pf_bytes = d->prefetch ? d->prefetch_bytes : 0;
  p.bits_out = (unsigned char*)d->relu_bits;
  MXDET_REQUIRE(!d->relu_bits || d->Cout % 8 == 0, MXDET_ESHAPE, "conv2d_fwd: relu_bits needs Cout %% 8 == 0");
  return launch<false>(p, as_stream(stream));
}

extern "C" int mxdet_conv2d_fwd_chain(const mxdet_conv_desc_t* d, const uint16_t* x, const uint16_t* w, const float* bias,
                                      const uint16_t* w2, const float* bias2, int32_t cout2, int32_t relu2,
                                      const uint16_t* residual2, uint16_t* y2, const uint16_t* w3, const float* bias3,
                                      int32_t cout3, int32_t relu3, uint16_t* y3, mxdet_stream_t stream) {
  clear_error();
  int rc = validate(d, "conv2d_fwd_chain");
  if (rc) return rc;
  MXDET_REQUIRE(d->KH == 3 && d->KW == 3 && d->stride == 1 && d->pad == 1, MXDET_ESHAPE,
                "conv2d_fwd_chain: the first convolution must be 3x3, stride 1, pad 1");
  MXDET_REQUIRE(d->Cin % 64 == 0 && d->Cout == 64 && cout2 == 256, MXDET_ESHAPE,
                "conv2d_fwd_chain: Cin %d must be a multiple of 64, Cout %d must be 64 and cout2 %d must be 256", d->Cin,
                d->Cout, cout2);
  MXDET_REQUIRE(!d->res_upsample && !d->relu_bits, MXDET_EINVAL, "conv2d_fwd_chain: no upsampled residual / relu_bits");
  MXDET_REQUIRE(x && w && w2 && y2, MXDET_EINVAL, "conv2d_fwd_chain: null pointer");
  MXDET_REQUIRE((long long)d->N * d->Ho * d->Wo * cout2 < (1ll << 31), MXDET_ESHAPE, "conv2d_fwd_chain: output exceeds 2^31");
  ConvP p;
  memset(&p, 0, sizeof(p));
  p.x = x; p.w = w; p.bias = bias; p.y = nullptr;
  p.N = d->N; p.Hs = d->H; p.Ws = d->W; p.C = d->Cin;
  p.Hd = d->Ho; p.Wd = d->Wo; p.Ncols = d->Cout;
  p.KH = 3; p.KW = 3; p.stride = 1; p.pad = 1;
  p.relu = d->relu;
  p.M = d->N * d->Ho * d->Wo;
  p.pf = d->prefetch; p.pf_bytes = d->prefetch ? d->prefetch_bytes : 0;
  p.chain_w = w2; p.chain_bias = bias2; p.chain_res = residual2; p.chain_y = y2; p.chain_relu = relu2;
  if (w3 != nullptr) {
    MXDET_REQUIRE(cout3 == 64 && y3 != nullptr, MXDET_ESHAPE, "conv2d_fwd_chain: the third convolution needs cout3 == 64 (got %d) and y3",
                  cout3);
    p.chain3_w = w3; p.chain3_bias = bias3; p.chain3_y = y3; p.chain3_relu = relu3;
  }
  return launch_cfg<128, 64, 4, 1, 2, false, false, 9, 256>(p, as_stream(stream));
}

namespace mxdet {
__global__ void __launch_bounds__(256)
conv_splitk_fold_kernel(const float* __restrict__ partial, int ksplit, long long M, int Ncols, const float* __restrict__ bias,
                        const uint16_t* __restrict__ res, int relu, uint16_t* __restrict__ y) {
  const long long i = ((long long)blockIdx.x * blockDim.x + threadIdx.x) * 8;
  const long long total = M * Ncols;
  if (i >= total) return;
  const int col = (int)(i % Ncols);
  float v[8];
  {
    const float4 a = *(const float4*)(partial + i), b = *(const float4*)(partial + i + 4);
    v[0] = a.x; v[1] = a.y; v[2] = a.z; v[3] = a.w; v[4] = b.x; v[5] = b.y; v[6] = b.z; v[7] = b.w;
  }
  for (int k = 1; k < ksplit; ++k) {
    const float4 a = *(const float4*)(partial + (size_t)k * total + i), b = *(const float4*)(partial + (size_t)k * total + i + 4);
    v[0] += a.x; v[1] += a.y; v[2] += a.z; v[3] += a.w; v[4] += b.x; v[5] += b.y; v[6] += b.z; v[7] += b.w;
  }
  if (bias) {
    const float4 a = *(const float4*)(bias + col), b = *(const float4*)(bias + col + 4);
    v[0] += a.x; v[1] += a.y; v[2] += a.z; v[3] += a.w; v[4] += b.x; v[5] += b.y; v[6] += b.z; v[7] += b.w;
  }
  if (res) {
    const uint4 rv = *(const uint4*)(res + i);
    v[0] += __uint_as_float(rv.x << 16); v[1] += __uint_as_float(rv.x & 0xffff0000u);
    v[2] += __uint_as_float(rv.y << 16); v[3] += __uint_as_float(rv.y & 0xffff0000u);
    v[4] += __uint_as_float(rv.z << 16); v[5] += __uint_as_float(rv.z & 0xffff0000u);
    v[6] += __uint_as_float(rv.w << 16); v[7] += __uint_as_float(rv.w & 0xffff0000u);
  }
  if (relu) {
#pragma unroll
    for (int k = 0; k < 8; ++k) v[k] = v[k] > 0.0f ? v[k] : 0.0f;
  }
  uint4 o;
  o.x = pack_bf16x2(v[0], v[1]); o.y = pack_bf16x2(v[2], v[3]); o.z = pack_bf16x2(v[4], v[5]); o.w = pack_bf16x2(v[6], v[7]);
  *(uint4*)(y + i) = o;
}
}

extern "C" size_t mxdet_conv2d_fwd_splitk_workspace_bytes(const mxdet_conv_desc_t* d, int32_t ksplit) {
  if (!d || ksplit < 1) return 0;
  return (size_t)ksplit * (size_t)d->N * d->Ho * d->Wo * d->Cout * sizeof(float);
}

extern "C" int mxdet_conv2d_fwd_splitk(const mxdet_conv_desc_t* d, const uint16_t* x, const uint16_t* w, const float* bias,
                                       const uint16_t* residual, uint16_t* y, int32_t ksplit, void* workspace,
                                       size_t workspace_bytes, mxdet_stream_t stream) {
  clear_error();
  int rc = validate(d, "conv2d_fwd_splitk");
  if (rc) return rc;
  MXDET_REQUIRE(d->KH == 1 && d->KW == 1 && d->stride == 1 && d->pad == 0 && !d->res_upsample, MXDET_ESHAPE,
                "conv2d_fwd_splitk: 1x1 / stride 1 / pad 0 layers (fully connected) only");
  MXDET_REQUIRE(d->Cin % 64 == 0 && d->Cout % 8 == 0, MXDET_ESHAPE, "conv2d_fwd_splitk: Cin %% 64, Cout %% 8");
  MXDET_REQUIRE(ksplit >= 1 && ksplit <= d->Cin / 64, MXDET_ESHAPE, "conv2d_fwd_splitk: 1 <= ksplit <= Cin / 64");
  MXDET_REQUIRE(x && w && y, MXDET_EINVAL, "conv2d_fwd_splitk: null pointer");
  if (ksplit == 1) return mxdet_conv2d_fwd(d, x, w, bias, residual, y, stream);
  const size_t need = mxdet_conv2d_fwd_splitk_workspace_bytes(d, ksplit);
  MXDET_REQUIRE(workspace && workspace_bytes >= need, MXDET_EWORKSPACE, "conv2d_fwd_splitk: workspace %zu < %zu", workspace_bytes, need);
  ConvP p;
  memset(&p, 0, sizeof(p));
  p.x = x; p.w = w; p.bias = nullptr; p.res = nullptr; p.mask = nullptr; p.y = y;
  p.N = d->N; p.Hs = d->H; p.Ws = d->W; p.C = d->Cin;
  p.Hd = d->Ho; p.Wd = d->Wo; p.Ncols = d->Cout;
  p.KH = 1; p.KW = 1; p.stride = 1; p.pad = 0;
  p.M = d->N * d->Ho * d->Wo;
  p.ksplit = ksplit; p.partial = (float*)workspace;
  const int big = (int)tuning(MXDET_TUNE_SPLITK_TILE);
  const int BT = big ? 128 : 64;
  const long long tiles = (long long)ceil_div(p.M, BT) * ceil_div(p.Ncols, BT);
  MXDET_REQUIRE(tiles % 8 == 0, MXDET_ESHAPE, "conv2d_fwd_splitk: the tile count (%lld) must be a multiple of 8", tiles);
  hipStream_t s = as_stream(stream);
  if (big == 1) rc = launch_cfg<128, 128, 2, 2, 2, false, false, 1>(p, s);
  else if (big == 2) rc = launch_cfg<128, 128, 2, 4, 2, false, false, 1>(p, s);
  else rc = launch_cfg<64, 64, 2, 2, 3, false, false, 1>(p, s);
  if (rc || route_probe_on()) return rc;
  const long long total = (long long)p.M * p.Ncols;
  hipLaunchKernelGGL(conv_splitk_fold_kernel, dim3((unsigned)ceil_div<long long>(total / 8, 256)), dim3(256), 0, s,
                     (const float*)workspace, ksplit, (long long)p.M, p.Ncols, bias, residual, d->relu, y);
  return check_launch("conv2d_fwd_splitk");
}

extern "C" int mxdet_conv2d_dgrad(const mxdet_conv_desc_t* d, const uint16_t* dy, const uint16_t* wt,
                                  const uint16_t* residual, const uint16_t* relu_mask, uint16_t* dx,
                                  mxdet_stream_t stream) {
  clear_error();
  int rc = validate(d, "conv2d_dgrad");
  if (rc) return rc;
  MXDET_REQUIRE(d->Cout % 64 == 0, MXDET_ESHAPE, "conv2d_dgrad: Cout %d must be a multiple of 64", d->Cout);
  MXDET_REQUIRE(d->Cin % 8 == 0, MXDET_ESHAPE, "conv2d_dgrad: Cin %d must be a multiple of 8", d->Cin);
  MXDET_REQUIRE(dy && wt && dx, MXDET_EINVAL, "conv2d_dgrad: null pointer");
  ConvP p;
  memset(&p, 0, sizeof(p));
  p.x = dy; p.w = wt; p.bias = nullptr; p.y = dx;
  p.res = residual ? residual : (d->accumulate ? dx : nullptr);
  p.mask = (d->relu && !d->relu_bits) ? relu_mask : nullptr;
  p.bits_in = d->relu ? (const unsigned char*)d->relu_bits : nullptr;
  MXDET_REQUIRE(!d->relu || relu_mask || d->relu_bits, MXDET_EINVAL, "conv2d_dgrad: relu set without relu_mask / relu_bits");
  p.N = d->N; p.Hs = d->Ho; p.Ws = d->Wo; p.C = d->Cout;
  p.Hd = d->H; p.Wd = d->W; p.Ncols = d->Cin;
  p.KH = d->KH; p.KW = d->KW; p.stride = d->stride; p.pad = d->pad;
  p.relu = 0; p.res_up = 0;
  p.M = d->N * d->H * d->W;
  p.pf = d->prefetch; p.pf_bytes = d->prefetch ? d->prefetch_bytes : 0;
  return launch<true>(p, as_stream(stream));
}

template <int BM, int BN, int WM, int WN, int NS, bool DGRAD>
static void launch_grouped_cfg(const ConvG* table, int n, int grid, hipStream_t s, int tapclass) {
  if (route_probe_on()) {
    const int32_t rec[kRouteWords] = {MXDET_ROUTE_CONV_GROUPED, BM, BN, WM, WN, NS, DGRAD, 0, tapclass == 1 ? 1 : tapclass == 2 ? 9 : 0,
                                      0, 0, 0, 0, 0, grid, n};
    route_record(rec);
    return;
  }
  if (tapclass == 1)
    hipLaunchKernelGGL((conv_igemm_grouped_kernel<BM, BN, WM, WN, NS, DGRAD, 1>), dim3((unsigned)grid), dim3(64 * WM * WN),
                       0, s, table, n);
  else if (tapclass == 2)
    hipLaunchKernelGGL((conv_igemm_grouped_kernel<BM, BN, WM, WN, NS, DGRAD, 9>), dim3((unsigned)grid), dim3(64 * WM * WN),
                       0, s, table, n);
  else
    hipLaunchKernelGGL((conv_igemm_grouped_kernel<BM, BN, WM, WN, NS, DGRAD>), dim3((unsigned)grid), dim3(64 * WM * WN),
                       0, s, table, n);
}

static const int kGroupedTiles[4][2] = {{128, 64}, {128, 128}, {64, 128}, {64, 64}};

extern "C" size_t mxdet_conv2d_grouped_table_bytes(int32_t n) { return n > 0 ? (size_t)n * sizeof(ConvG) : 0; }

extern "C" int mxdet_conv2d_grouped_plan(const mxdet_conv_item_t* items, int32_t n, int32_t kind, void* table_host,
                                         size_t table_bytes, int32_t* cfg_out, int32_t* grid_out) {
  clear_error();
  MXDET_REQUIRE(items && n > 0 && table_host && cfg_out && grid_out, MXDET_EINVAL, "conv2d_grouped_plan: null pointer");
  MXDET_REQUIRE(kind == 0 || kind == 1, MXDET_EINVAL, "conv2d_grouped_plan: kind must be 0 (forward) or 1 (dgrad)");
  MXDET_REQUIRE(table_bytes >= (size_t)n * sizeof(ConvG), MXDET_EWORKSPACE, "conv2d_grouped_plan: table too small");
  ConvG* t = (ConvG*)table_host;
  long long t64 = 0, t128_max = 0;
  int max_cols = 0, kmax = 0;
  int tapclass = -1;
  for (int i = 0; i < n; ++i) {
    const mxdet_conv_desc_t* d = &items[i].desc;
    int rc = validate(d, "conv2d_grouped_plan");
    if (rc) return rc;
    ConvP& p = t[i].p;
    memset(&t[i], 0, sizeof(ConvG));
    MXDET_REQUIRE(items[i].src && items[i].filt && items[i].dst, MXDET_EINVAL, "conv2d_grouped_plan: item %d: null pointer", i);
    if (kind == 0) {
      MXDET_REQUIRE(d->Cin % 64 == 0 && d->Cout % 8 == 0, MXDET_ESHAPE, "conv2d_grouped_plan: item %d: Cin %% 64, Cout %% 8", i);
      p.x = (const uint16_t*)items[i].src; p.w = (const uint16_t*)items[i].filt; p.bias = items[i].bias;
      p.res = (const uint16_t*)items[i].residual; p.mask = nullptr; p.y = (uint16_t*)items[i].dst;
      p.bits_out = (unsigned char*)d->relu_bits;
      p.N = d->N; p.Hs = d->H; p.Ws = d->W; p.C = d->Cin;
      p.Hd = d->Ho; p.Wd = d->Wo; p.Ncols = d->Cout;
      p.relu = d->relu; p.res_up = d->res_upsample;
      p.M = d->N * d->Ho * d->Wo;
    } else {
      MXDET_REQUIRE(d->Cout % 64 == 0 && d->Cin % 8 == 0, MXDET_ESHAPE, "conv2d_grouped_plan: item %d: Cout %% 64, Cin %% 8", i);
      MXDET_REQUIRE(d->stride == 1, MXDET_ESHAPE, "conv2d_grouped_plan: item %d: strided data gradients are not grouped", i);
      MXDET_REQUIRE(!d->relu || items[i].relu_mask || d->relu_bits, MXDET_EINVAL, "conv2d_grouped_plan: item %d: relu without mask", i);
      p.x = (const uint16_t*)items[i].src; p.w = (const uint16_t*)items[i].filt; p.bias = nullptr;
      p.y = (uint16_t*)items[i].dst;
      p.res = items[i].residual ? (const uint16_t*)items[i].residual : (d->accumulate ? (const uint16_t*)items[i].dst : nullptr);
      p.mask = (d->relu && !d->relu_bits) ? (const uint16_t*)items[i].relu_mask : nullptr;
      p.bits_in = d->relu ? (const unsigned char*)d->relu_bits : nullptr;
      p.N = d->N; p.Hs = d->Ho; p.Ws = d->Wo; p.C = d->Cout;
      p.Hd = d->H; p.Wd = d->W; p.Ncols = d->Cin;
      p.relu = 0; p.res_up = 0;
      p.M = d->N * d->H * d->W;
    }
    p.KH = d->KH; p.KW = d->KW; p.stride = d->stride; p.pad = d->pad;
    p.pf = d->prefetch; p.pf_bytes = d->prefetch ? d->prefetch_bytes : 0;
    {
      const int tc = (d->stride != 1 && (kind == 1 || d->KH * d->KW == 1)) ? 0
                     : (d->KH == 1 && d->KW == 1 && d->pad == 0) ? 1 : (d->KH == 3 && d->KW == 3 && d->pad == 1) ? 2 : 0;
      tapclass = tapclass < 0 ? tc : (tapclass == tc ? tc : 0);
    }
    t64 += (long long)ceil_div(p.M, 64) * ceil_div(p.Ncols, 128);
    long long t128 = (long long)ceil_div(p.M, 128) * ceil_div(p.Ncols, 128);
    t128_max = t128 > t128_max ? t128 : t128_max;
    max_cols = p.Ncols > max_cols ? p.Ncols : max_cols;
    kmax = p.KH * p.KW * p.C > kmax ? p.KH * p.KW * p.C : kmax;
  }
  int cfg;
  if (max_cols <= 64) cfg = 0;
  else if (t128_max >= thr_t128() && kmax > 256) cfg = 1;
  else if (t64 >= thr_t64()) cfg = 2;
  else cfg = 3;
  const int BM = kGroupedTiles[cfg][0], BN = kGroupedTiles[cfg][1];
  long long blocks = 0;
  for (int i = 0; i < n; ++i) {
    ConvP& p = t[i].p;
    p.tiles_m = ceil_div(p.M, BM);
    p.tiles_n = ceil_div(p.Ncols, BN);
    t[i].nblocks = p.tiles_m * p.tiles_n;
    t[i].block0 = (int)blocks;
    blocks += (long long)align_up((size_t)t[i].nblocks, 8);
    MXDET_REQUIRE(blocks < (1ll << 30), MXDET_ESHAPE, "conv2d_grouped_plan: group too large");
  }
  if (tuning(MXDET_TUNE_STATIC_TAPS) == 0 || tapclass < 0) tapclass = 0;
  *cfg_out = cfg + 4 * tapclass;
  *grid_out = (int32_t)blocks;
  return MXDET_OK;
}

extern "C" int mxdet_conv2d_grouped(const void* table_dev, int32_t n, int32_t kind, int32_t cfg, int32_t grid,
                                    mxdet_stream_t stream) {
  clear_error();
  MXDET_REQUIRE(table_dev && n > 0 && grid > 0, MXDET_EINVAL, "conv2d_grouped: empty group");
  MXDET_REQUIRE((kind == 0 || kind == 1) && cfg >= 0 && cfg <= 11, MXDET_EINVAL, "conv2d_grouped: bad kind / cfg");
  const ConvG* t = (const ConvG*)table_dev;
  hipStream_t s = as_stream(stream);
  const int tc = cfg >> 2;
  cfg &= 3;
  if (kind == 0) {
    switch (cfg) {
      case 0: launch_grouped_cfg<128, 64, 4, 1, 2, false>(t, n, grid, s, tc); break;
      case 1: launch_grouped_cfg<128, 128, 2, 2, 2, false>(t, n, grid, s, tc); break;
      case 2: launch_grouped_cfg<64, 128, 2, 2, 2, false>(t, n, grid, s, tc); break;
      default: launch_grouped_cfg<64, 64, 2, 2, 3, false>(t, n, grid, s, tc); break;
    }
  } else {
    switch (cfg) {
      case 0: launch_grouped_cfg<128, 64, 4, 1, 2, true>(t, n, grid, s, tc); break;
      case 1: launch_grouped_cfg<128, 128, 2, 2, 2, true>(t, n, grid, s, tc); break;
      case 2: launch_grouped_cfg<64, 128, 2, 2, 2, true>(t, n, grid, s, tc); break;
      default: launch_grouped_cfg<64, 64, 2, 2, 3, true>(t, n, grid, s, tc); break;
    }
  }
  if (route_probe_on()) return MXDET_OK;
  return check_launch("conv2d_grouped");
}
```

mxdetection_amd/models/backbones/resnet.py:

```python
import os

import torch

from ...ops import dense
from ..utils.layers import ConvLayer, DeformConvLayer, cached_buf


BITMASKS = os.environ.get("MXDET_TUNE_RELU_BITS", "1") == "1"
CHAIN_FROZEN = os.environ.get("MXDET_TUNE_CHAIN", "1") != "0"
CHAIN3_FROZEN = os.environ.get("MXDET_TUNE_CHAIN", "2") not in ("0", "1")


class Bottleneck:
    def __init__(self, name, cin, planes, stride, downsample, trainable, need_dx, arena, ws, device, gen, dcn=None):
        kw = dict(arena=arena, ws=ws, device=device, gen=gen, trainable=trainable, train_bias=False)
        self.trainable, self.need_dx = trainable, need_dx
        self.conv3 = ConvLayer(name + ".conv3", planes, planes * 4, 1, init_std=0.25 * (2.0 / planes) ** 0.5, **kw)
        self.dcn = dcn is not None
        if self.dcn:
            assert trainable, "deformable convolutions only in trainable stages"
            self.conv2 = DeformConvLayer(name + ".conv2", planes, planes, stride, dcn["groups"], dcn["modulated"],
                                         arena=arena, ws=ws, device=device, gen=gen)
        else:
            self.conv2 = ConvLayer(name + ".conv2", planes, planes, 3, stride, **kw)
        self.conv1 = ConvLayer(name + ".conv1", cin, planes, 1, **kw)
        self.down = ConvLayer(name + ".down", cin, planes * 4, 1, stride, 0, **kw) if downsample else None
        self.x = self.a1 = self.a2 = self.y = self.sc = None
        self.bufs = {}
        self.y_key = "y"

    def layers(self):
        c2 = self.conv2.layers() if self.dcn else [self.conv2]
        return [l for l in [self.conv3] + c2 + [self.conv1, self.down] if l is not None]

    def _buf(self, key, shape):
        return cached_buf(self.bufs, key, shape, torch.bfloat16, self.conv1.device)

    def plan(self, x_shape):
        s1 = self.conv1.out_shape(x_shape)
        s2 = self.conv2.out_shape(s1)
        self.conv1.plan(x_shape)
        self.conv2.plan(s1)
        self.conv3.plan(s2)
        if self.down is not None:
            self.down.plan(x_shape)
        return self.conv3.out_shape(s2)

    def _bits(self, key, shape):
        return cached_buf(self.bufs, key, shape[:3] + (shape[3] // 8,), torch.uint8, self.conv1.device)

    def chainable(self):
        return (CHAIN_FROZEN and not self.trainable and self.conv2.stride == 1 and self.conv2.cout == 64 and
                self.conv3.cout == 256)

    def forward(self, x, x_bits=None, a1_ready=False, next_block=None):
        self.x, self.x_bits = x, x_bits
        bits = self.trainable and BITMASKS
        a1 = self._buf("a1", self.conv1.out_shape(x.shape))
        s2 = self.conv2.out_shape(a1.shape)
        oshape = self.conv3.out_shape(s2)
        self.a1_bits = self._bits("a1b", a1.shape) if bits else None
        self.a2_bits = self._bits("a2b", s2) if bits else None
        self.y_bits = self._bits("yb", oshape) if bits else None
        if self.down is None:
            if not a1_ready:
                self.a1 = self.conv1.forward(x, relu=True, out=a1, bits_out=self.a1_bits)
            sc = x
        else:
            sc = self._buf("sc", oshape)
            dense.conv2d_group("fwd", [self.conv1.fwd_call(x, relu=True, out=a1, bits_out=self.a1_bits),
                                       self.down.fwd_call(x, out=sc)], self.conv1.device)
            self.a1 = a1
        if self.chainable():
            if dense.PF_TRACE is not None:
                dense.PF_TRACE.append((self.conv2, "f", dense.mem_range(self.conv3.w_bf16, self.conv2.w_bf16), None))
            self.a2 = None
            nb = next_block
            kw = {}
            if nb is not None:
                nb.a1 = nb._buf("a1", nb.conv1.out_shape(oshape))
                kw = dict(w3=nb.conv1.w_bf16, bias3=nb.conv1.bias_f32, relu3=True, out3=nb.a1)
            r = dense.conv2d_forward_chain(self.a1, self.conv2.w_bf16, self.conv2.bias_f32, self.conv3.w_bf16,
                                           self.conv3.bias_f32, sc, relu=True, relu2=True, out=self._buf(self.y_key, oshape),
                                           prefetch=self.conv2.pf_fwd, **kw)
            self.y = r[0] if nb is not None else r
            return self.y
        self.a2 = self.conv2.forward(self.a1, relu=True, out=self._buf("a2", s2), bits_out=self.a2_bits)
        self.y = self.conv3.forward(self.a2, relu=True, residual=sc, out=self._buf(self.y_key, oshape), bits_out=self.y_bits)
        return self.y

    def backward(self, ds, dx_buf, dx_has_grad):
        c1, c2, c3 = self.conv1, self.conv2, self.conv3
        c3.backward_weight(self.a2, ds)
        d_a2 = c3.backward_data(ds, self.a2.shape, relu_mask=self.a2, out=self._buf("d_a2", self.a2.shape),
                                relu_bits=self.a2_bits)
        c2.backward_weight(self.a1, d_a2)
        d_a1 = c2.backward_data(d_a2, self.a1.shape, relu_mask=self.a1, out=self._buf("d_a1", self.a1.shape),
                                relu_bits=self.a1_bits)
        c1.backward_weight(self.x, d_a1)
        if self.down is not None:
            self.down.backward_weight(self.x, ds)
        if not self.need_dx:
            return None
        xb = self.x_bits
        if self.down is not None:
            self.down.backward_data(ds, self.x.shape, accumulate=dx_has_grad, out=dx_buf)
            c1.backward_data(d_a1, self.x.shape, residual=dx_buf, relu_mask=self.x, out=dx_buf, relu_bits=xb)
        else:
            if dx_has_grad:
                dense.add_bf16(dx_buf, ds, dx_buf)
                c1.backward_data(d_a1, self.x.shape, residual=dx_buf, relu_mask=self.x, out=dx_buf, relu_bits=xb)
            else:
                c1.backward_data(d_a1, self.x.shape, residual=ds, relu_mask=self.x, out=dx_buf, relu_bits=xb)
        return dx_buf


class ResNet:

    def __init__(self, depth, arena, ws, device, gen, frozen_stages=1, dcn_stages=(), dcn_modulated=True, dcn_groups=1):
        blocks = {50: (3, 4, 6, 3), 101: (3, 4, 23, 3)}[depth]
        self.device = device
        dcn_stages = set(int(s) for s in dcn_stages)
        bad = [s for s in dcn_stages if s not in (3, 4, 5) or s - 2 < max(1, frozen_stages)]
        if bad:
            raise ValueError("dcn_stages %s: only trainable stages among 3, 4, 5" % sorted(bad))
        self.dcn_stages = sorted(dcn_stages)
        dcn = {"groups": int(dcn_groups), "modulated": bool(dcn_modulated)}
        self.stages = [None] * 4
        cins = [64, 256, 512, 1024]
        for si in (3, 2, 1, 0):
            planes = 64 << si
            trainable = si > frozen_stages - 1 and si >= 1 if frozen_stages >= 1 else True
            stage = []
            for bi in reversed(range(blocks[si])):
                cin = cins[si] if bi == 0 else planes * 4
                stride = 2 if (bi == 0 and si > 0) else 1
                need_dx = trainable and not (bi == 0 and (si == 0 or si - 1 < frozen_stages))
                stage.insert(0, Bottleneck("layer%d.%d" % (si + 1, bi), cin, planes, stride, bi == 0, trainable,
                                           need_dx, arena, ws, device, gen,
                                           dcn=dcn if si + 2 in dcn_stages else None))
            self.stages[si] = stage
        self.stem_w = (torch.randn((64, 7, 7, 3), generator=gen) * (2.0 / 147) ** 0.5).to(torch.bfloat16).to(device)
        self.stem_b = torch.zeros((64,), dtype=torch.float32, device=device)
        self.bufs = {}
        self.outs = None
        self.front_override = None
        self.eager_parity = 0
        self.front_outs = []

    def layers(self):
        return [l for st in self.stages for b in st for l in b.layers()]

    def plan(self, image_shape):
        N, _, H, W = image_shape
        s = (N, ((H - 1) // 2 + 1 - 1) // 2 + 1, ((W - 1) // 2 + 1 - 1) // 2 + 1, 64)
        shapes = []
        for st in self.stages:
            for b in st:
                s = b.plan(s)
            shapes.append(s)
        return shapes

    def forward(self, image):
        if self.front_override is not None:
            return self.forward_rest(self.front_override)
        return self.forward_rest(self.forward_front(image, self.eager_parity))

    def frozen_front(self):
        n = 0
        for st in self.stages:
            if any(b.trainable for b in st):
                break
            n += 1
        return n

    def forward_front(self, image, parity=0):
        N, _, H, W = image.shape
        H1, W1 = (H - 1) // 2 + 1, (W - 1) // 2 + 1
        dev = self.stem_w.device
        x = dense.stem_conv7x7_pool(image, self.stem_w, self.stem_b,
                                    cached_buf(self.bufs, "pool", (N, (H1 - 1) // 2 + 1, (W1 - 1) // 2 + 1, 64),
                                               torch.bfloat16, dev))
        nf = self.frozen_front()
        if nf > 0:
            self.stages[nf - 1][-1].y_key = "y%d" % parity if parity else "y"
        self.front_outs = []
        for st in self.stages[:nf]:
            x = self._stage_forward(st, x, None)
            self.front_outs.append(x)
        return x

    def _stage_forward(self, st, x, xb):
        ready = False
        for i, b in enumerate(st):
            nb = st[i + 1] if i + 1 < len(st) else None
            ride = (CHAIN3_FROZEN and nb is not None and b.chainable() and nb.chainable() and nb.down is None and
                    nb.conv1.cout == 64 and nb.conv1.stride == 1)
            x = b.forward(x, xb, a1_ready=ready, next_block=nb if ride else None)
            ready = ride
            xb = b.y_bits
        self._xb = xb
        return x

    def forward_rest(self, x):
        nf = self.frozen_front()
        if self.front_override is None:
            outs = list(self.front_outs[:nf])
        else:
            outs = ([None] * (nf - 1) + [x]) if nf else []
        xb = None
        for st in self.stages[nf:]:
            x = self._stage_forward(st, x, xb)
            xb = self._xb
            outs.append(x)
        self.outs = outs
        return outs

    def backward(self, dC):
        for si in (3, 2, 1):
            stage = self.stages[si]
            if not stage[0].trainable:
                break
            ds = dC[si]
            for bi in reversed(range(len(stage))):
                b = stage[bi]
                if bi > 0:
                    dxb = b._buf("dx", b.x.shape)
                    ds = b.backward(ds, dxb, False)
                else:
                    if b.need_dx:
                        ds = b.backward(ds, dC[si - 1], True)
                    else:
                        b.backward(ds, None, False)
```

mxdetection_amd/models/utils/layers.py:

```python
import contextlib
import os
import math

import torch

from ...ops import dense


def cached_buf(bufs, key, shape, dtype, device, zero=False):
    k = (key, tuple(shape), dtype)
    b = bufs.get(k)
    if b is None:
        b = (torch.zeros if zero else torch.empty)(tuple(shape), dtype=dtype, device=device)
        bufs[k] = b
    return b


class Workspace:

    def __init__(self, device):
        self.device = device
        self.need = 0
        self.buf = None
        self._retired = []
        self.side = None
        self.grouping = False
        self.pending = []
        self.plans = {}
        self.gbuf = None

    def defer(self, layer, x, dy):
        self.pending.append((layer, x, dy))

    def flush(self):
        if not self.pending:
            return
        items, self.pending = self.pending, []
        if "wgrad" in os.environ.get("MXDET_ABL_SKIP", ""):
            return
        key = tuple((id(l), x.data_ptr(), dy.data_ptr()) for l, x, dy in items)
        plan = self.plans.get(key)
        capturing = torch.cuda.is_current_stream_capturing()
        if plan is None and not capturing:
            calls = [(x, dy, l.k, l.k, l.stride, l.pad, l.arena.view(l.wi, "g"),
                      l.arena.view(l.bi, "g") if l.train_bias else None, False) for l, x, dy in items]
            plan = dense.GroupedWgrad(calls, self.device)
            self.plans[key] = plan
            if self.gbuf is None or self.gbuf.numel() < plan.workspace_bytes:
                self._retired.append(self.gbuf)
                self.gbuf = torch.empty((max(plan.workspace_bytes, 256),), dtype=torch.uint8, device=self.device)
        ctx = self.fork()
        with (ctx if ctx is not None else contextlib.nullcontext()):
            if plan is None or self.gbuf is None or self.gbuf.numel() < plan.workspace_bytes:
                for l, x, dy in items:
                    dense.conv2d_wgrad(x, dy, l.k, l.k, l.stride, l.pad, l.arena.view(l.wi, "g"),
                                       l.arena.view(l.bi, "g") if l.train_bias else None, False, self.get())
            else:
                plan.launch(self.gbuf)
    def fork(self):
        if self.side is None:
            return None
        self.side.wait_stream(torch.cuda.current_stream())
        return torch.cuda.stream(self.side)

    def join(self):
        if self.side is not None:
            torch.cuda.current_stream().wait_stream(self.side)

    def require(self, nbytes):
        self.need = max(self.need, int(nbytes))

    def get(self):
        if self.buf is None or self.buf.numel() < self.need:
            self._retired.append(self.buf)
            self.buf = torch.empty((self.need,), dtype=torch.uint8, device=self.device)
        return self.buf


class ParamArena:
    def __init__(self, device):
        self.device = device
        self.entries = []
        self.size = 0
        self.w = self.g = self.m = self.wb = None

    def register(self, name, shape):
        n = 1
        for s in shape:
            n *= s
        off = self.size
        self.entries.append((name, tuple(shape), off, n))
        self.size += (n + 63) // 64 * 64
        return len(self.entries) - 1

    def finalize(self):
        dev = self.device
        self.w = torch.zeros((self.size,), dtype=torch.float32, device=dev)
        self.g = torch.zeros((self.size,), dtype=torch.float32, device=dev)
        self.m = torch.zeros((self.size,), dtype=torch.float32, device=dev)
        self.wb = torch.zeros((self.size,), dtype=torch.bfloat16, device=dev)

    def view(self, idx, which):
        _, shape, off, n = self.entries[idx]
        return getattr(self, which)[off:off + n].view(shape)

    def offset_of(self, idx):
        return self.entries[idx][2]

    def refresh_bf16(self):
        dense.f32_to_bf16(self.w, self.wb)

    def sgd_step(self, lr, momentum, wd, rescale):
        dense.sgd_momentum_update(self.w, self.g, self.m, self.wb, lr, momentum, wd, rescale)


class ConvLayer:

    def __init__(self, name, cin, cout, k, stride=1, pad=None, bias=True, trainable=True, arena=None, ws=None,
                 device="cuda", gen=None, init_std=None, zero_init=False, train_bias=True, cout_real=None):
        self.name, self.cin, self.cout, self.k, self.stride = name, cin, cout, k, stride
        self.pad = (k // 2) if pad is None else pad
        self.trainable = trainable
        self.arena, self.ws = arena, ws
        self.has_bias = bias
        std = init_std if init_std is not None else math.sqrt(2.0 / (k * k * cin))
        w0 = torch.zeros((cout, k, k, cin)) if zero_init else torch.randn((cout, k, k, cin), generator=gen) * std
        self.cout_real = cout if cout_real is None else cout_real
        if self.cout_real < cout:
            w0[self.cout_real:] = 0
        self._w0 = w0
        self.train_bias = bias and trainable and train_bias
        self.frozen_bias = None
        if bias and not self.train_bias:
            self.frozen_bias = torch.zeros((cout,), dtype=torch.float32, device=device)
        if trainable:
            self.wi = arena.register(name + ".weight", (cout, k, k, cin))
            self.bi = arena.register(name + ".bias", (cout,)) if self.train_bias else None
        else:
            self.w_bf16 = w0.to(torch.bfloat16).to(device)
            self.bias_f32 = self.frozen_bias
        self.wt = None
        self.device = device
        self.pf_fwd = self.pf_bwd = None

    def materialize(self):
        if not self.trainable:
            return
        self.arena.view(self.wi, "w").copy_(self._w0.to(self.device))
        self.w_bf16 = self.arena.view(self.wi, "wb")
        self.bias_f32 = self.arena.view(self.bi, "w") if self.train_bias else self.frozen_bias
        self.wt = torch.empty((self.cin, self.k, self.k, self.cout), dtype=torch.bfloat16, device=self.device)
        self._w0 = None

    def plan(self, x_shape):
        if self.trainable:
            self.ws.require(dense.conv2d_wgrad_workspace_bytes(x_shape, self.cout, self.k, self.k, self.stride, self.pad))

    def out_shape(self, x_shape):
        N, H, W, _ = x_shape
        return (N, (H + 2 * self.pad - self.k) // self.stride + 1, (W + 2 * self.pad - self.k) // self.stride + 1,
                self.cout)

    def refresh_transposed(self):
        if self.trainable:
            dense.filter_transpose(self.w_bf16, self.wt)

    def forward(self, x, relu=False, residual=None, res_upsample=False, out=None, bits_out=None):
        if dense.PF_TRACE is not None:
            dense.PF_TRACE.append((self, "f", dense.mem_range(self.w_bf16), None))
        return dense.conv2d_forward(x, self.w_bf16, self.bias_f32, residual, self.stride, self.pad, relu, res_upsample,
                                    out, prefetch=self.pf_fwd, bits_out=bits_out)

    def fwd_call(self, x, relu=False, residual=None, res_upsample=False, out=None, bits_out=None):
        t = (x, self.w_bf16, self.bias_f32, residual, self.stride, self.pad, relu, res_upsample, out)
        return t if bits_out is None else t + (bits_out,)

    def dgrad_call(self, dy, x_shape, residual=None, relu_mask=None, accumulate=False, out=None, relu_bits=None):
        t = (dy, self.wt, tuple(x_shape), self.k, self.k, self.stride, self.pad, residual, relu_mask, accumulate, out)
        return t if relu_bits is None else t + (relu_bits,)

    def backward_data(self, dy, x_shape, residual=None, relu_mask=None, accumulate=False, out=None, relu_bits=None):
        if dense.PF_TRACE is not None:
            dense.PF_TRACE.append((self, "b", dense.mem_range(self.wt), None))
        return dense.conv2d_dgrad(dy, self.wt, x_shape, self.k, self.k, self.stride, self.pad, residual,
                                  None if relu_bits is not None else relu_mask, accumulate, out, prefetch=self.pf_bwd,
                                  relu_bits=relu_bits)

    def backward_weight(self, x, dy, accumulate=False):
        if self.ws.grouping and not accumulate:
            self.ws.defer(self, x, dy)
            return
        dw = self.arena.view(self.wi, "g")
        db = self.arena.view(self.bi, "g") if self.train_bias else None
        ctx = self.ws.fork()
        if ctx is None:
            dense.conv2d_wgrad(x, dy, self.k, self.k, self.stride, self.pad, dw, db, accumulate, self.ws.get())
        else:
            with ctx:
                dense.conv2d_wgrad(x, dy, self.k, self.k, self.stride, self.pad, dw, db, accumulate, self.ws.get())


class GroupNormLayer:
    trainable = True

    def __init__(self, name, channels, groups, arena, device="cuda", eps=1e-5):
        if groups <= 0 or channels % groups or (channels // groups) % 8:
            raise ValueError("GroupNorm %s: %d groups do not divide %d channels into multiples of 8" % (name, groups, channels))
        self.name, self.C, self.G, self.eps = name, channels, groups, eps
        self.arena, self.device = arena, device
        self.gi = arena.register(name + ".gamma", (channels,))
        self.bi = arena.register(name + ".beta", (channels,))
        self.bufs = {}
        self.plans = {}
        self.gamma = self.beta = None
        self.x = self.y = self.mean = self.rstd = None
        self.relu = False

    def materialize(self):
        self.gamma, self.beta = self.arena.view(self.gi, "w"), self.arena.view(self.bi, "w")
        self.gamma.fill_(1.0)
        self.beta.zero_()

    def named_params(self):
        return [(self.name + ".gamma", self.gi), (self.name + ".beta", self.bi)]

    def plan(self, x_shape):
        x_shape = tuple(x_shape)
        p = self.plans.get(x_shape)
        if p is None:
            from ...ops import group_norm as GN
            stats = [cached_buf(self.bufs, k, (x_shape[0], self.G), torch.float32, self.device) for k in ("mean", "rstd")]
            ws = [cached_buf(self.bufs, "ws%d" % b, (max(GN.workspace_bytes(x_shape, self.G, bool(b)), 256),), torch.uint8,
                             self.device) for b in (0, 1)]
            p = self.plans[x_shape] = (stats[0], stats[1], ws[0], ws[1])
        return p

    def forward(self, x, relu=False, out=None):
        from ...ops import group_norm as GN
        mean, rstd, ws, _ = self.plan(x.shape)
        y, _, _ = GN.group_norm_forward(x, self.gamma, self.beta, self.G, self.eps, relu, out=out, mean=mean, rstd=rstd,
                                        workspace=ws)
        self.x, self.y, self.mean, self.rstd, self.relu = x, y, mean, rstd, relu
        return y

    def backward(self, dy, out=None):
        from ...ops import group_norm as GN
        return GN.group_norm_backward(self.x, dy, self.mean, self.rstd, self.gamma, self.G, self.arena.view(self.gi, "g"),
                                      self.arena.view(self.bi, "g"), y=None, beta=self.beta, eps=self.eps, relu=self.relu,
                                      out=out, workspace=self.plan(self.x.shape)[3])


class DeformConvLayer:

    def __init__(self, name, cin, cout, stride=1, groups=1, modulated=True, arena=None, ws=None, device="cuda", gen=None,
                 train_bias=False):
        self.name, self.cin, self.cout, self.stride, self.pad = name, cin, cout, stride, 1
        self.groups, self.modulated = groups, bool(modulated)
        self.k = 3
        self.trainable = True
        self.conv = ConvLayer(name, 9 * cin, cout, 1, 1, 0, arena=arena, ws=ws, device=device, gen=gen,
                              train_bias=train_bias)
        self.conv.dcn_khwc = (3, 3, cin)
        nreal = (27 if self.modulated else 18) * groups
        self.offset = ConvLayer(name + "_offset", cin, (nreal + 63) // 64 * 64, 3, stride, 1, arena=arena, ws=ws,
                                device=device, gen=gen, zero_init=True, cout_real=nreal)
        self.ws = ws
        self.device = device
        self.bufs = {}
        self.x = self.off = self.col = None

    def layers(self):
        return [self.conv, self.offset]

    def _buf(self, key, shape, dtype=torch.bfloat16):
        return cached_buf(self.bufs, key, shape, dtype, self.device)

    def out_shape(self, x_shape):
        return self.offset.out_shape(x_shape)[:3] + (self.cout,)

    def plan(self, x_shape):
        N, Ho, Wo, _ = self.out_shape(x_shape)
        self.offset.plan(x_shape)
        self.conv.plan((N, Ho, Wo, 9 * self.cin))

    def forward(self, x, relu=False, residual=None, out=None, bits_out=None):
        from ...ops import deform_conv
        N, Ho, Wo, _ = self.out_shape(x.shape)
        off = self.offset.forward(x, out=self._buf("off", (N, Ho, Wo, self.offset.cout)))
        col = deform_conv.im2col(x, off, self.stride, self.pad, self.groups, self.modulated,
                                 out=self._buf("col", (N, Ho, Wo, 9 * self.cin)))
        self.x, self.off, self.col = x, off, col
        return self.conv.forward(col, relu=relu, residual=residual, out=out, bits_out=bits_out)

    def backward_weight(self, x, dy, accumulate=False):
        self.conv.backward_weight(self.col, dy, accumulate)

    def backward_data(self, dy, x_shape, residual=None, relu_mask=None, accumulate=False, out=None, relu_bits=None):
        from ...ops import deform_conv
        assert residual is None and not accumulate, "DeformConvLayer.backward_data: no residual / accumulate"
        x_shape = tuple(x_shape)
        dcol = self.conv.backward_data(dy, self.col.shape, out=self._buf("dcol", self.col.shape))
        a = (self.stride, self.pad, self.groups, self.modulated)
        doff = deform_conv.col2im_coord(self.x, self.off, dcol, *a, out=self._buf("doff", self.off.shape))
        nws = deform_conv.col2im_workspace_bytes(x_shape, *a, self.off.shape[3])
        dxu = deform_conv.col2im(self.off, dcol, x_shape, *a, out=self._buf("dxu", x_shape),
                                 workspace=self._buf("c2i_ws", (max(nws, 256),), torch.uint8))
        self.offset.backward_weight(self.x, doff)
        return self.offset.backward_data(doff, x_shape, residual=dxu, relu_mask=relu_mask, out=out, relu_bits=relu_bits)
```

mxdetection_amd/ops/dense.py:

```python
import ctypes as C

import torch

from .. import _lib
from .._lib import ConvDescT, check, ptr, stream_ptr

_DT = {torch.float32: 0, torch.bfloat16: 1}


def mem_range(*tensors):
    spans = [(t.data_ptr(), t.numel() * t.element_size()) for t in tensors]
    bases = {t.untyped_storage().data_ptr() for t in tensors}
    if len(bases) == 1:
        lo = min(p for p, _ in spans)
        hi = max(p + n for p, n in spans)
        if hi - lo <= 2 * sum(n for _, n in set(spans)):
            return (lo, hi - lo)
    return spans[0]


def conv_desc(N, H, W, Cin, Cout, KH, KW, stride, pad, relu=False, res_upsample=False, accumulate=False, prefetch=None,
              relu_bits=None):
    d = ConvDescT()
    if relu_bits is not None:
        d.relu_bits = relu_bits.data_ptr()
    if prefetch is not None:
        d.prefetch, d.prefetch_bytes = prefetch if isinstance(prefetch, tuple) else mem_range(prefetch)
    d.N, d.H, d.W, d.Cin, d.Cout, d.KH, d.KW, d.stride, d.pad = N, H, W, Cin, Cout, KH, KW, stride, pad
    d.Ho = (H + 2 * pad - KH) // stride + 1
    d.Wo = (W + 2 * pad - KW) // stride + 1
    d.relu, d.res_upsample, d.accumulate = int(relu), int(res_upsample), int(accumulate)
    return d


def conv2d_forward(x, w, bias=None, residual=None, stride=1, pad=0, relu=False, res_upsample=False, out=None, prefetch=None,
                   bits_out=None):
    lib = _lib.load()
    N, H, W, Cin = x.shape
    Cout, KH, KW, _ = w.shape
    d = conv_desc(N, H, W, Cin, Cout, KH, KW, stride, pad, relu, res_upsample, prefetch=prefetch, relu_bits=bits_out)
    if out is None:
        out = torch.empty((N, d.Ho, d.Wo, Cout), dtype=torch.bfloat16, device=x.device)
    check(lib.mxdet_conv2d_fwd(C.byref(d), ptr(x), ptr(w), ptr(bias), ptr(residual), ptr(out), stream_ptr()),
          "conv2d_fwd")
    return out


def conv2d_forward_splitk(x, w, bias=None, residual=None, relu=False, ksplit=4, out=None, workspace=None):
    lib = _lib.load()
    N, H, W, Cin = x.shape
    Cout = w.shape[0]
    d = conv_desc(N, H, W, Cin, Cout, 1, 1, 1, 0, relu, False)
    if out is None:
        out = torch.empty((N, d.Ho, d.Wo, Cout), dtype=torch.bfloat16, device=x.device)
    need = lib.mxdet_conv2d_fwd_splitk_workspace_bytes(C.byref(d), ksplit)
    if workspace is None or workspace.numel() < need:
        workspace = torch.empty((need,), dtype=torch.uint8, device=x.device)
    check(lib.mxdet_conv2d_fwd_splitk(C.byref(d), ptr(x), ptr(w), ptr(bias), ptr(residual), ptr(out), ksplit, ptr(workspace),
                                      workspace.numel(), stream_ptr()), "conv2d_fwd_splitk")
    return out


def conv2d_forward_chain(x, w, bias, w2, bias2=None, residual2=None, relu=True, relu2=True, out=None, prefetch=None,
                         w3=None, bias3=None, relu3=True, out3=None):
    lib = _lib.load()
    N, H, W, Cin = x.shape
    Cmid, Cout2 = w.shape[0], w2.shape[0]
    d = conv_desc(N, H, W, Cin, Cmid, 3, 3, 1, 1, relu, False, prefetch=prefetch)
    if out is None:
        out = torch.empty((N, H, W, Cout2), dtype=torch.bfloat16, device=x.device)
    if w3 is not None and out3 is None:
        out3 = torch.empty((N, H, W, w3.shape[0]), dtype=torch.bfloat16, device=x.device)
    check(lib.mxdet_conv2d_fwd_chain(C.byref(d), ptr(x), ptr(w), ptr(bias), ptr(w2), ptr(bias2), Cout2, int(relu2),
                                     ptr(residual2), ptr(out), ptr(w3), ptr(bias3), 0 if w3 is None else w3.shape[0],
                                     int(relu3), ptr(out3), stream_ptr()), "conv2d_fwd_chain")
    return out if w3 is None else (out, out3)


def conv2d_dgrad(dy, wt, x_shape, KH, KW, stride=1, pad=0, residual=None, relu_mask=None, accumulate=False, out=None,
                 prefetch=None, relu_bits=None):
    lib = _lib.load()
    N, H, W, Cin = x_shape
    Cout = dy.shape[3]
    d = conv_desc(N, H, W, Cin, Cout, KH, KW, stride, pad, relu=(relu_mask is not None or relu_bits is not None),
                  accumulate=accumulate, prefetch=prefetch, relu_bits=relu_bits)
    if out is None:
        out = torch.empty(tuple(x_shape), dtype=torch.bfloat16, device=dy.device)
    check(lib.mxdet_conv2d_dgrad(C.byref(d), ptr(dy), ptr(wt), ptr(residual), ptr(relu_mask), ptr(out), stream_ptr()),
          "conv2d_dgrad")
    return out


def conv2d_wgrad_workspace_bytes(x_shape, Cout, KH, KW, stride, pad):
    N, H, W, Cin = x_shape
    d = conv_desc(N, H, W, Cin, Cout, KH, KW, stride, pad)
    return _lib.load().mxdet_conv2d_wgrad_workspace_bytes(C.byref(d))


def conv2d_wgrad(x, dy, KH, KW, stride=1, pad=0, dw=None, db=None, accumulate=False, workspace=None):
    lib = _lib.load()
    N, H, W, Cin = x.shape
    Cout = dy.shape[3]
    d = conv_desc(N, H, W, Cin, Cout, KH, KW, stride, pad, accumulate=accumulate)
    need = lib.mxdet_conv2d_wgrad_workspace_bytes(C.byref(d))
    if workspace is None:
        workspace = torch.empty((need,), dtype=torch.uint8, device=x.device)
    if dw is None:
        dw = torch.empty((Cout, KH, KW, Cin), dtype=torch.float32, device=x.device)
    check(lib.mxdet_conv2d_wgrad(C.byref(d), ptr(x), ptr(dy), ptr(dw), ptr(db), ptr(workspace), workspace.numel(),
                                 stream_ptr()), "conv2d_wgrad")
    return dw


class GroupedConv:

    def __init__(self, kind, calls, device, hint=None):
        lib = _lib.load()
        n = len(calls)
        items = (_lib.ConvItemT * n)()
        self.keep, self.kind = calls, 0 if kind == "fwd" else 1
        self.flops = 0.0
        dp = lambda t: None if t is None else t.data_ptr()
        for it, c in zip(items, calls):
            if self.kind == 0:
                x, w, bias, residual, stride, pad, relu, res_up, out = c[:9]
                bits = c[9] if len(c) > 9 else None
                N, H, W, Cin = x.shape
                Cout, KH, KW, _ = w.shape
                it.desc = conv_desc(N, H, W, Cin, Cout, KH, KW, stride, pad, relu, res_up, prefetch=hint, relu_bits=bits)
                hint = None
                it.src, it.filt, it.bias, it.residual, it.relu_mask, it.dst = dp(x), dp(w), dp(bias), dp(residual), None, dp(out)
                self.flops += 2.0 * N * it.desc.Ho * it.desc.Wo * Cout * KH * KW * Cin
            else:
                dy, wt, x_shape, KH, KW, stride, pad, residual, relu_mask, accumulate, out = c[:11]
                bits = c[11] if len(c) > 11 else None
                N, H, W, Cin = x_shape
                Cout = dy.shape[3]
                it.desc = conv_desc(N, H, W, Cin, Cout, KH, KW, stride, pad, relu=(relu_mask is not None or bits is not None),
                                    accumulate=accumulate, prefetch=hint, relu_bits=bits)
                hint = None
                it.src, it.filt, it.bias, it.residual, it.relu_mask, it.dst = (dp(dy), dp(wt), None, dp(residual),
                                                                              None if bits is not None else dp(relu_mask), dp(out))
                self.flops += 2.0 * N * dy.shape[1] * dy.shape[2] * Cout * KH * KW * Cin
        nbytes = lib.mxdet_conv2d_grouped_table_bytes(n)
        host = (C.c_ubyte * nbytes)()
        cfg, grid = C.c_int32(0), C.c_int32(0)
        check(lib.mxdet_conv2d_grouped_plan(items, n, self.kind, host, nbytes, C.byref(cfg), C.byref(grid)),
              "conv2d_grouped_plan")
        self.table = torch.frombuffer(bytearray(host), dtype=torch.uint8).clone().to(device)
        self.n, self.cfg, self.grid = n, cfg.value, grid.value

    def launch(self):
        check(_lib.load().mxdet_conv2d_grouped(ptr(self.table), self.n, self.kind, self.cfg, self.grid, stream_ptr()),
              "conv2d_grouped")


_group_plans = {}


PF_TRACE = None
GROUP_HINTS = {}


def conv2d_group(kind, calls, device):
    key = (kind,) + tuple(tuple(t.data_ptr() if torch.is_tensor(t) else t for t in c) for c in calls)
    if PF_TRACE is not None and calls:
        PF_TRACE.append((None, "g", mem_range(*[c[1] for c in calls]), key if len(calls) > 1 else None))
    if len(calls) == 1:
        plan = None
    else:
        plan = _group_plans.get(key)
        if plan is None and not torch.cuda.is_current_stream_capturing():
            plan = GroupedConv(kind, calls, device, GROUP_HINTS.get(key))
            _group_plans[key] = plan
    if plan is not None:
        plan.launch()
        return
    for c in calls:
        if kind == "fwd":
            x, w, bias, residual, stride, pad, relu, res_up, out = c[:9]
            conv2d_forward(x, w, bias, residual, stride, pad, relu, res_up, out, bits_out=c[9] if len(c) > 9 else None)
        else:
            dy, wt, x_shape, KH, KW, stride, pad, residual, relu_mask, accumulate, out = c[:11]
            conv2d_dgrad(dy, wt, x_shape, KH, KW, stride, pad, residual, relu_mask, accumulate, out,
                         relu_bits=c[11] if len(c) > 11 else None)


class GroupedWgrad:

    def __init__(self, calls, device):
        lib = _lib.load()
        n = len(calls)
        items = (_lib.WgradItemT * n)()
        self.keep = calls
        self.flops = 0.0
        self.heaviest = (0.0, "")
        for it, (x, dy, KH, KW, stride, pad, dw, db, accumulate) in zip(items, calls):
            N, H, W, Cin = x.shape
            it.desc = conv_desc(N, H, W, Cin, dy.shape[3], KH, KW, stride, pad, accumulate=accumulate)
            it.x, it.dy, it.dw, it.db = x.data_ptr(), dy.data_ptr(), dw.data_ptr(), (db.data_ptr() if db is not None else None)
            fl = 2.0 * dy.shape[0] * dy.shape[1] * dy.shape[2] * dy.shape[3] * KH * KW * Cin
            self.flops += fl
            if fl > self.heaviest[0]:
                self.heaviest = (fl, "N=%d %dx%d %d->%d %dx%d" % (N, H, W, Cin, dy.shape[3], KH, KW))
        nbytes = lib.mxdet_conv2d_wgrad_grouped_table_bytes(n)
        host = (C.c_ubyte * nbytes)()
        ws, gw, gb, gr = C.c_size_t(0), C.c_int32(0), C.c_int32(0), C.c_int32(0)
        check(lib.mxdet_conv2d_wgrad_grouped_plan(items, n, host, nbytes, C.byref(ws), C.byref(gw), C.byref(gb),
                                                  C.byref(gr)), "conv2d_wgrad_grouped_plan")
        self.grid_big = gb.value
        self.table = torch.frombuffer(bytearray(host), dtype=torch.uint8).clone().to(device)
        self.n, self.grid_wgrad, self.grid_reduce, self.workspace_bytes = n, gw.value, gr.value, ws.value

    def launch(self, workspace):
        check(_lib.load().mxdet_conv2d_wgrad_grouped(ptr(self.table), self.n, self.grid_wgrad, self.grid_big, self.grid_reduce,
                                                     ptr(workspace), workspace.numel() if workspace is not None else 0,
                                                     self.workspace_bytes, stream_ptr()), "conv2d_wgrad_grouped")


def filter_transpose(w, out=None):
    lib = _lib.load()
    Cout, KH, KW, Cin = w.shape
    if out is None:
        out = torch.empty((Cin, KH, KW, Cout), dtype=torch.bfloat16, device=w.device)
    check(lib.mxdet_filter_transpose(ptr(w), Cout, KH, KW, Cin, ptr(out), stream_ptr()), "filter_transpose")
    return out


def make_transpose_table(pairs, device):
    import struct
    buf = bytearray()
    tile0 = 0
    for w, wt in pairs:
        Cout, KH, KW, Cin = w.shape
        buf += struct.pack("<QQiiii", w.data_ptr(), wt.data_ptr(), Cout, KH * KW, Cin, tile0)
        tile0 += ((Cin + 63) // 64) * ((Cout + 63) // 64) * KH * KW
    table = torch.frombuffer(buf, dtype=torch.uint8).clone().to(device)
    return table, len(pairs), tile0


def filter_transpose_batched(table, ndesc, total_tiles):
    check(_lib.load().mxdet_filter_transpose_batched(ptr(table), ndesc, total_tiles, stream_ptr()),
          "filter_transpose_batched")


def stem_conv7x7(image, w, bias=None, out=None):
    lib = _lib.load()
    N, _, H, W = image.shape
    Ho, Wo = (H - 1) // 2 + 1, (W - 1) // 2 + 1
    if out is None:
        out = torch.empty((N, Ho, Wo, 64), dtype=torch.bfloat16, device=image.device)
    check(lib.mxdet_stem_conv7x7(ptr(image), _DT[image.dtype], N, H, W, ptr(w), ptr(bias), ptr(out), stream_ptr()),
          "stem_conv7x7")
    return out


def stem_conv7x7_pool(image, w, bias=None, out=None):
    lib = _lib.load()
    N, _, H, W = image.shape
    Ho, Wo = (H - 1) // 2 + 1, (W - 1) // 2 + 1
    Hp, Wp = (Ho - 1) // 2 + 1, (Wo - 1) // 2 + 1
    if out is None:
        out = torch.empty((N, Hp, Wp, 64), dtype=torch.bfloat16, device=image.device)
    check(lib.mxdet_stem_conv7x7_pool(ptr(image), _DT[image.dtype], N, H, W, ptr(w), ptr(bias), ptr(out), stream_ptr()),
          "stem_conv7x7_pool")
    return out


def maxpool3x3s2(x, out=None):
    lib = _lib.load()
    N, H, W, Cc = x.shape
    Ho, Wo = (H - 1) // 2 + 1, (W - 1) // 2 + 1
    if out is None:
        out = torch.empty((N, Ho, Wo, Cc), dtype=torch.bfloat16, device=x.device)
    check(lib.mxdet_maxpool3x3s2(ptr(x), N, H, W, Cc, ptr(out), stream_ptr()), "maxpool3x3s2")
    return out


def subsample2(x, out=None):
    lib = _lib.load()
    N, H, W, Cc = x.shape
    if out is None:
        out = torch.empty((N, (H + 1) // 2, (W + 1) // 2, Cc), dtype=torch.bfloat16, device=x.device)
    check(lib.mxdet_subsample2(ptr(x), N, H, W, Cc, ptr(out), stream_ptr()), "subsample2")
    return out


def subsample2_backward(dy, dx, accumulate=False):
    lib = _lib.load()
    N, H, W, Cc = dx.shape
    check(lib.mxdet_subsample2_bwd(ptr(dy), N, H, W, Cc, int(accumulate), ptr(dx), stream_ptr()), "subsample2_bwd")
    return dx


def upsample2_backward(dfine, dcoarse, accumulate=False):
    lib = _lib.load()
    N, Hf, Wf, Cc = dfine.shape
    check(lib.mxdet_upsample2_bwd(ptr(dfine), N, Hf, Wf, Cc, int(accumulate), ptr(dcoarse), stream_ptr()),
          "upsample2_bwd")
    return dcoarse


def pixel_shuffle2_inv_relu(dy_up, act, out=None):
    R, H, W, C4 = act.shape
    if out is None:
        out = torch.empty_like(act)
    check(_lib.load().mxdet_pixel_shuffle2_inv_relu(ptr(dy_up), ptr(act), R, H, W, C4 // 4, ptr(out), stream_ptr()),
          "pixel_shuffle2_inv_relu")
    return out


def pixel_shuffle2(x, out=None, inverse=False):
    lib = _lib.load()
    if not inverse:
        R, H, W, C4 = x.shape
        Cc = C4 // 4
        if out is None:
            out = torch.empty((R, 2 * H, 2 * W, Cc), dtype=torch.bfloat16, device=x.device)
    else:
        R, H2, W2, Cc = x.shape
        H, W = H2 // 2, W2 // 2
        if out is None:
            out = torch.empty((R, H, W, 4 * Cc), dtype=torch.bfloat16, device=x.device)
    check(lib.mxdet_pixel_shuffle2(ptr(x), R, H, W, Cc, int(inverse), ptr(out), stream_ptr()), "pixel_shuffle2")
    return out


def add_bf16(a, b, out=None):
    lib = _lib.load()
    if out is None:
        out = torch.empty_like(a)
    check(lib.mxdet_add_bf16(ptr(a), ptr(b), a.numel(), ptr(out), stream_ptr()), "add_bf16")
    return out


def relu_backward(dy, y, out=None):
    lib = _lib.load()
    if out is None:
        out = torch.empty_like(dy)
    check(lib.mxdet_relu_bwd_bf16(ptr(dy), ptr(y), dy.numel(), ptr(out), stream_ptr()), "relu_bwd_bf16")
    return out


def relu_forward(x, out=None):
    return relu_backward(x, x, out)


def f32_to_bf16(x, out=None):
    lib = _lib.load()
    if out is None:
        out = torch.empty(x.shape, dtype=torch.bfloat16, device=x.device)
    check(lib.mxdet_f32_to_bf16(ptr(x), x.numel(), ptr(out), stream_ptr()), "f32_to_bf16")
    return out


def f32_accum_to_bf16(x, y, accumulate):
    check(_lib.load().mxdet_f32_accum_to_bf16(ptr(x), x.numel(), int(accumulate), ptr(y), stream_ptr()),
          "f32_accum_to_bf16")
    return y


def nchw_to_nhwc(x):
    lib = _lib.load()
    N, Cc, H, W = x.shape
    out = torch.empty((N, H, W, Cc), dtype=torch.bfloat16, device=x.device)
    check(lib.mxdet_nchw_to_nhwc_bf16(ptr(x), _DT[x.dtype], N, Cc, H, W, ptr(out), stream_ptr()), "nchw_to_nhwc_bf16")
    return out


def nhwc_to_nchw(x):
    lib = _lib.load()
    N, H, W, Cc = x.shape
    out = torch.empty((N, Cc, H, W), dtype=torch.float32, device=x.device)
    check(lib.mxdet_nhwc_to_nchw_f32(ptr(x), N, Cc, H, W, ptr(out), stream_ptr()), "nhwc_to_nchw_f32")
    return out


def sgd_momentum_update(w, grad, mom, w_bf16, lr, momentum=0.9, wd=1e-4, rescale=1.0):
    if torch.is_tensor(lr):
        check(_lib.load().mxdet_sgd_momentum_update_sched(ptr(w), ptr(grad), ptr(mom), ptr(w_bf16), w.numel(), ptr(lr),
                                                          momentum, wd, rescale, stream_ptr()), "sgd_momentum_update_sched")
        return
    check(_lib.load().mxdet_sgd_momentum_update(ptr(w), ptr(grad), ptr(mom), ptr(w_bf16), w.numel(), lr, momentum, wd,
                                                rescale, stream_ptr()), "sgd_momentum_update")
```

Before: 450.7 images/sec.

## Compute downsample dgrad compactly and fuse it into conv1 dgrad epilogue

In bottleneck blocks with a stride-2 1x1 downsample, the downsample data gradient is now computed as a stride-1 1x1 GEMM on the compact output grid, grouped with conv3's dgrad in one launch. It reads the existing upstream gradient at a pixel stride and writes a quarter-size buffer. conv1's dgrad epilogue then adds this compact result at even pixels, through a new RES2 kernel variant that handles sub-sampled or strided residuals. This removes the separate full-resolution strided dgrad pass and its read-modify-write of dx. The cost is extra index arithmetic in the epilogue, and the r2 route is excluded from the large-tile configs.

```diff
diff --git a/include/mxdet.h b/include/mxdet.h
--- a/include/mxdet.h
+++ b/include/mxdet.h
@@ -191,6 +191,8 @@
   const void* prefetch;
   int64_t prefetch_bytes;
   void* relu_bits;
+  int32_t res_stride, res_h, res_w;
+  const void* res_sub;
 } mxdet_conv_desc_t;
 
 int mxdet_conv2d_fwd(const mxdet_conv_desc_t* d, const uint16_t* x, const uint16_t* w,
diff --git a/include/mxdet_debug.h b/include/mxdet_debug.h
--- a/include/mxdet_debug.h
+++ b/include/mxdet_debug.h
@@ -41,6 +41,8 @@
 #define MXDET_ROUTE_WGRAD 2
 #define MXDET_ROUTE_CONV_GROUPED 3
 #define MXDET_ROUTE_WGRAD_GROUPED 4
+#define MXDET_ROUTE_RES_SUB 1
+#define MXDET_ROUTE_RES_STRIDED 2
 #define MXDET_ROUTE_WORDS 16
 #define MXDET_ROUTE_MAX 4
 int mxdet_debug_route_probe(int32_t on);
diff --git a/mxdetection_amd/_lib.py b/mxdetection_amd/_lib.py
--- a/mxdetection_amd/_lib.py
+++ b/mxdetection_amd/_lib.py
@@ -49,6 +49,7 @@
         ("Ho", c_i32), ("Wo", c_i32),
         ("relu", c_i32), ("res_upsample", c_i32), ("accumulate", c_i32),
         ("prefetch", c_vp), ("prefetch_bytes", c_i64), ("relu_bits", c_vp),
+        ("res_stride", c_i32), ("res_h", c_i32), ("res_w", c_i32), ("res_sub", c_vp),
     ]
 
 
diff --git a/mxdetection_amd/csrc/conv.hip b/mxdetection_amd/csrc/conv.hip
--- a/mxdetection_amd/csrc/conv.hip
+++ b/mxdetection_amd/csrc/conv.hip
@@ -31,6 +31,8 @@
   unsigned char* bits_out;
   const unsigned char* bits_in;
   int force_cfg;
+  int res_stride, res_h, res_w;
+  const uint16_t* res_sub;
   const uint16_t* chain_w;
   const float* chain_bias;
   const uint16_t* chain_res;
@@ -56,7 +58,7 @@
 #define MXDET_CS(k) do { } while (0)
 #endif
 
-template <int BM, int BN, int WM, int WN, int NS, bool DGRAD, bool PAR = false, int TAPS = 0, int CHAIN = 0>
+template <int BM, int BN, int WM, int WN, int NS, bool DGRAD, bool PAR = false, int TAPS = 0, int CHAIN = 0, bool RES2 = false>
 __device__ __forceinline__ void conv_igemm_tile(const ConvP& p, int bid, const int nwg) {
   constexpr int NW = WM * WN, NTHR = 64 * NW;
   constexpr int WTM = BM / WM, WTN = BN / WN;
@@ -69,6 +71,7 @@
   static_assert(MT % 2 == 0, "epilogue stages two m-tiles at a time");
   static_assert(NS >= 2 && (NS - 2) * (GA + GB) <= 63, "vmcnt is a 6-bit counter");
   static_assert(TAPS == 0 || ((TAPS == 1 || TAPS == 9) && !PAR), "static taps: 1x1 or 3x3");
+  static_assert(!RES2 || (DGRAD && TAPS == 1 && CHAIN == 0), "strided / sub-sampled residual: stride-1 1x1 data gradient");
   constexpr int EP_STRIDE = WTN + 4;
   constexpr int EP_BYTES = NW * 32 * EP_STRIDE * 4;
   constexpr int MAIN_BYTES = NBUF * STAGE * 2;
@@ -609,7 +612,32 @@
       oks[ps] = rowok && colok;
       pixs[ps] = oks[ps] ? pix : 0;
     }
-    if (e_res) {
+    if constexpr (RES2) {
+      const int Hc = (p.Hd + 1) >> 1, Wc = (p.Wd + 1) >> 1;
+      const bool any_res = p.res_sub != nullptr || e_res != nullptr;
+#pragma unroll
+      for (int ps = 0; ps < PASSES; ++ps) {
+        if (!any_res) { rres[ps] = make_uint4(0u, 0u, 0u, 0u); continue; }
+        const int m = (int)pixs[ps], c = oks[ps] ? col : 0;
+        int img, hd, wd, rem;
+        if (smallm) {
+          img = fast_divmod(m, hw_d, rcp_hw, &rem);
+          hd = fast_divmod(rem, p.Wd, rcp_w, &wd);
+        } else {
+          img = m / hw_d; rem = m - img * hw_d;
+          hd = rem / p.Wd; wd = rem - hd * p.Wd;
+        }
+        const bool sub = p.res_sub != nullptr && ((hd | wd) & 1) == 0;
+        const size_t ri_sub = ((size_t)(img * Hc + (hd >> 1)) * Wc + (wd >> 1)) * e_ncols + c;
+        const size_t ri_res = p.res_stride > 1
+                                  ? ((size_t)(img * p.res_h + hd * p.res_stride) * p.res_w + wd * p.res_stride) * e_ncols + c
+                                  : pixs[ps] * e_ncols + c;
+        const bool none = !sub && e_res == nullptr;
+        const uint16_t* rp = (sub || none) ? p.res_sub : e_res;
+        rres[ps] = *(const uint4*)(rp + (sub ? ri_sub : none ? (size_t)0 : ri_res));
+        if (none) rres[ps] = make_uint4(0u, 0u, 0u, 0u);
+      }
+    } else if (e_res) {
 #pragma unroll
       for (int ps = 0; ps < PASSES; ++ps) {
         size_t ri = pixs[ps] * e_ncols + (oks[ps] ? col : 0);
@@ -658,7 +686,7 @@
         }
       }
       float v[8] = {v0.x + b0.x, v0.y + b0.y, v0.z + b0.z, v0.w + b0.w, v1.x + b1.x, v1.y + b1.y, v1.z + b1.z, v1.w + b1.w};
-      if (e_res) {
+      if (RES2 || e_res) {
         const uint4 rv = rres[ps];
         v[0] += __uint_as_float(rv.x << 16); v[1] += __uint_as_float(rv.x & 0xffff0000u);
         v[2] += __uint_as_float(rv.y << 16); v[3] += __uint_as_float(rv.y & 0xffff0000u);
@@ -735,10 +763,10 @@
 #endif
 }
 
-template <int BM, int BN, int WM, int WN, int NS, bool DGRAD, bool PAR = false, int TAPS = 0, int CHAIN = 0>
+template <int BM, int BN, int WM, int WN, int NS, bool DGRAD, bool PAR = false, int TAPS = 0, int CHAIN = 0, bool RES2 = false>
 __global__ void __launch_bounds__(64 * WM * WN)
 conv_igemm_kernel(ConvP p) {
-  conv_igemm_tile<BM, BN, WM, WN, NS, DGRAD, PAR, TAPS, CHAIN>(p, (int)blockIdx.x, (int)gridDim.x);
+  conv_igemm_tile<BM, BN, WM, WN, NS, DGRAD, PAR, TAPS, CHAIN, RES2>(p, (int)blockIdx.x, (int)gridDim.x);
 }
 
 struct ConvG {
@@ -746,7 +774,7 @@
   int block0, nblocks;
 };
 
-template <int BM, int BN, int WM, int WN, int NS, bool DGRAD, int TAPS = 0>
+template <int BM, int BN, int WM, int WN, int NS, bool DGRAD, int TAPS = 0, bool RES2 = false>
 __global__ void __launch_bounds__(64 * WM * WN)
 conv_igemm_grouped_kernel(const ConvG* __restrict__ table, int n) {
   int lo = 0, hi = n - 1;
@@ -759,7 +787,7 @@
   const int nb = table[lo].nblocks;
   if (b >= nb) return;
   const ConvP p = table[lo].p;
-  conv_igemm_tile<BM, BN, WM, WN, NS, DGRAD, false, TAPS>(p, b, nb);
+  conv_igemm_tile<BM, BN, WM, WN, NS, DGRAD, false, TAPS, 0, RES2>(p, b, nb);
 }
 
 static thread_local int g_force_cfg = 0;
@@ -768,8 +796,14 @@
 static int thr_t128() { return (int)tuning(MXDET_TUNE_T128); }
 static int thr_par64() { return (int)tuning(MXDET_TUNE_PAR64); }
 
-template <int BM, int BN, int WM, int WN, int NS, bool DGRAD, bool PAR = false, int TAPS = 0, int CHAIN = 0>
+static int res2_flags(const ConvP& p) {
+  return (p.res_sub != nullptr ? MXDET_ROUTE_RES_SUB : 0) | (p.res_stride > 1 ? MXDET_ROUTE_RES_STRIDED : 0);
+}
+
+template <int BM, int BN, int WM, int WN, int NS, bool DGRAD, bool PAR = false, int TAPS = 0, int CHAIN = 0, bool RES2 = false>
 static int launch_cfg(ConvP& p, hipStream_t s) {
+  MXDET_REQUIRE(RES2 || res2_flags(p) == 0, MXDET_EINVAL,
+                "conv2d: a strided / sub-sampled residual needs the stride-1 1x1 data-gradient route");
   if (PAR) {
     int t = 0;
     for (int c = 0; c < 4; ++c) {
@@ -785,11 +819,11 @@
   if (TAPS == 1 && p.ksplit > 1) nwg *= p.ksplit;
   if (route_probe_on()) {
     const int32_t rec[kRouteWords] = {MXDET_ROUTE_CONV, BM, BN, WM, WN, NS, DGRAD, PAR, TAPS, CHAIN, p.tiles_m, p.tiles_n,
-                                      p.m_begin, p.ksplit, (int32_t)nwg, 0};
+                                      p.m_begin, p.ksplit, (int32_t)nwg, res2_flags(p)};
     route_record(rec);
     return MXDET_OK;
   }
-  hipLaunchKernelGGL((conv_igemm_kernel<BM, BN, WM, WN, NS, DGRAD, PAR, TAPS, CHAIN>), dim3((unsigned)nwg),
+  hipLaunchKernelGGL((conv_igemm_kernel<BM, BN, WM, WN, NS, DGRAD, PAR, TAPS, CHAIN, RES2>), dim3((unsigned)nwg),
                      dim3(64 * WM * WN), 0, s, p);
   return check_launch("conv2d");
 }
@@ -820,8 +854,10 @@
   const int taps = p.KH * p.KW;
   const int st = ((p.stride != 1 && (DGRAD || taps == 1)) || tuning(MXDET_TUNE_STATIC_TAPS) == 0) ? 0
                  : (taps == 1 && p.pad == 0) ? 1 : (p.KH == 3 && p.KW == 3 && p.pad == 1) ? 9 : 0;
+  const bool r2 = DGRAD && st == 1 && res2_flags(p) != 0;
 #define MXDET_LAUNCH_ST(BM, BN, WM, WN, NS)                                                        \
-  (st == 1 ? launch_cfg<BM, BN, WM, WN, NS, DGRAD, false, 1>(p, s)                                 \
+  (r2 ? launch_cfg<BM, BN, WM, WN, NS, DGRAD, false, 1, 0, DGRAD>(p, s)                            \
+   : st == 1 ? launch_cfg<BM, BN, WM, WN, NS, DGRAD, false, 1>(p, s)                               \
            : st == 9 ? launch_cfg<BM, BN, WM, WN, NS, DGRAD, false, 9>(p, s)                       \
                      : launch_cfg<BM, BN, WM, WN, NS, DGRAD>(p, s))
   if constexpr (DGRAD) {
@@ -838,7 +874,7 @@
     }
   }
   if (p.Ncols <= 64) return MXDET_LAUNCH_ST(128, 64, 4, 1, 2);
-  if (t128 >= thr_t128() && K > 256) {
+  if (t128 >= thr_t128() && K > 256 && !r2) {
     const int tn = ceil_div(p.Ncols, 256);
     const long long full = (long long)(p.M / 256) * tn;
     const long long rounds = full / 256;
@@ -858,7 +894,7 @@
   }
   {
     const long long t256 = (long long)(p.M / 256) * (p.Ncols / 256);
-    if (p.M % 256 == 0 && p.Ncols % 256 == 0 && t256 >= 160 && t256 <= 256 && K >= 1024 && p.m_begin == 0)
+    if (p.M % 256 == 0 && p.Ncols % 256 == 0 && t256 >= 160 && t256 <= 256 && K >= 1024 && p.m_begin == 0 && !r2)
       return launch_cfg<256, 256, 2, 4, 2, DGRAD>(p, s);
   }
   if (st != 0 && p.Ncols >= 128 && t128 >= tuning(MXDET_TUNE_T128W)) return MXDET_LAUNCH_ST(128, 128, 2, 4, 2);
@@ -879,6 +915,23 @@
   MXDET_REQUIRE((long long)d->N * d->H * d->W * d->Cin < (1ll << 31) &&
                     (long long)d->N * d->Ho * d->Wo * d->Cout < (1ll << 31),
                 MXDET_ESHAPE, "%s: tensor exceeds 2^31 elements", who);
+  return MXDET_OK;
+}
+
+static int set_res2(const mxdet_conv_desc_t* d, const void* residual, ConvP& p, const char* who) {
+  if (d->res_stride <= 1 && d->res_sub == nullptr) return MXDET_OK;
+  MXDET_REQUIRE(d->KH == 1 && d->KW == 1 && d->stride == 1 && d->pad == 0, MXDET_ESHAPE,
+                "%s: res_stride / res_sub are for 1x1, stride 1, pad 0 data gradients", who);
+  if (d->res_stride > 1) {
+    MXDET_REQUIRE(residual != nullptr, MXDET_EINVAL, "%s: res_stride needs a residual operand", who);
+    MXDET_REQUIRE(d->res_h >= (d->H - 1) * d->res_stride + 1 && d->res_w >= (d->W - 1) * d->res_stride + 1, MXDET_ESHAPE,
+                  "%s: a %d x %d residual read with pixel stride %d does not cover %d x %d", who, d->res_h, d->res_w,
+                  d->res_stride, d->H, d->W);
+    MXDET_REQUIRE((long long)d->N * d->res_h * d->res_w * d->Cin < (1ll << 31), MXDET_ESHAPE,
+                  "%s: strided residual exceeds 2^31 elements", who);
+    p.res_stride = d->res_stride; p.res_h = d->res_h; p.res_w = d->res_w;
+  }
+  p.res_sub = (const uint16_t*)d->res_sub;
   return MXDET_OK;
 }
 
@@ -1055,18 +1108,23 @@
   p.relu = 0; p.res_up = 0;
   p.M = d->N * d->H * d->W;
   p.pf = d->prefetch; p.pf_bytes = d->prefetch ? d->prefetch_bytes : 0;
+  rc = set_res2(d, residual, p, "conv2d_dgrad");
+  if (rc) return rc;
   return launch<true>(p, as_stream(stream));
 }
 
 template <int BM, int BN, int WM, int WN, int NS, bool DGRAD>
-static void launch_grouped_cfg(const ConvG* table, int n, int grid, hipStream_t s, int tapclass) {
+static void launch_grouped_cfg(const ConvG* table, int n, int grid, hipStream_t s, int tapclass, int r2flags) {
   if (route_probe_on()) {
     const int32_t rec[kRouteWords] = {MXDET_ROUTE_CONV_GROUPED, BM, BN, WM, WN, NS, DGRAD, 0, tapclass == 1 ? 1 : tapclass == 2 ? 9 : 0,
-                                      0, 0, 0, 0, 0, grid, n};
+                                      0, 0, tapclass, r2flags, 0, grid, n};
     route_record(rec);
     return;
   }
-  if (tapclass == 1)
+  if (DGRAD && tapclass == 1 && r2flags != 0)
+    hipLaunchKernelGGL((conv_igemm_grouped_kernel<BM, BN, WM, WN, NS, DGRAD, 1, DGRAD>), dim3((unsigned)grid), dim3(64 * WM * WN),
+                       0, s, table, n);
+  else if (tapclass == 1)
     hipLaunchKernelGGL((conv_igemm_grouped_kernel<BM, BN, WM, WN, NS, DGRAD, 1>), dim3((unsigned)grid), dim3(64 * WM * WN),
                        0, s, table, n);
   else if (tapclass == 2)
@@ -1091,6 +1149,7 @@
   long long t64 = 0, t128_max = 0;
   int max_cols = 0, kmax = 0;
   int tapclass = -1;
+  int r2flags = 0;
   for (int i = 0; i < n; ++i) {
     const mxdet_conv_desc_t* d = &items[i].desc;
     int rc = validate(d, "conv2d_grouped_plan");
@@ -1120,12 +1179,16 @@
       p.Hd = d->H; p.Wd = d->W; p.Ncols = d->Cin;
       p.relu = 0; p.res_up = 0;
       p.M = d->N * d->H * d->W;
+      rc = set_res2(d, items[i].residual, p, "conv2d_grouped_plan");
+      if (rc) return rc;
+      r2flags |= res2_flags(p);
     }
     p.KH = d->KH; p.KW = d->KW; p.stride = d->stride; p.pad = d->pad;
     p.pf = d->prefetch; p.pf_bytes = d->prefetch ? d->prefetch_bytes : 0;
     {
-      const int tc = (d->stride != 1 && (kind == 1 || d->KH * d->KW == 1)) ? 0
-                     : (d->KH == 1 && d->KW == 1 && d->pad == 0) ? 1 : (d->KH == 3 && d->KW == 3 && d->pad == 1) ? 2 : 0;
+      const int tc = (d->stride != 1 && kind == 1) ? 0
+                     : (d->KH == 1 && d->KW == 1 && d->pad == 0) ? 1
+                     : (d->KH == 3 && d->KW == 3 && d->pad == 1 && (d->stride == 1 || kind == 0)) ? 2 : 0;
       tapclass = tapclass < 0 ? tc : (tapclass == tc ? tc : 0);
     }
     t64 += (long long)ceil_div(p.M, 64) * ceil_div(p.Ncols, 128);
@@ -1151,7 +1214,9 @@
     MXDET_REQUIRE(blocks < (1ll << 30), MXDET_ESHAPE, "conv2d_grouped_plan: group too large");
   }
   if (tuning(MXDET_TUNE_STATIC_TAPS) == 0 || tapclass < 0) tapclass = 0;
-  *cfg_out = cfg + 4 * tapclass;
+  MXDET_REQUIRE(r2flags == 0 || tapclass == 1, MXDET_ESHAPE,
+                "conv2d_grouped_plan: a strided / sub-sampled residual needs a group of stride-1 1x1 data gradients");
+  *cfg_out = cfg + 4 * tapclass + 16 * r2flags;
   *grid_out = (int32_t)blocks;
   return MXDET_OK;
 }
@@ -1160,24 +1225,25 @@
                                     mxdet_stream_t stream) {
   clear_error();
   MXDET_REQUIRE(table_dev && n > 0 && grid > 0, MXDET_EINVAL, "conv2d_grouped: empty group");
-  MXDET_REQUIRE((kind == 0 || kind == 1) && cfg >= 0 && cfg <= 11, MXDET_EINVAL, "conv2d_grouped: bad kind / cfg");
+  MXDET_REQUIRE((kind == 0 || kind == 1) && cfg >= 0 && cfg <= 63, MXDET_EINVAL, "conv2d_grouped: bad kind / cfg");
   const ConvG* t = (const ConvG*)table_dev;
   hipStream_t s = as_stream(stream);
-  const int tc = cfg >> 2;
+  const int tc = (cfg >> 2) & 3, r2 = cfg >> 4;
+  MXDET_REQUIRE(tc <= 2 && (r2 == 0 || (kind == 1 && tc == 1)), MXDET_EINVAL, "conv2d_grouped: bad cfg");
   cfg &= 3;
   if (kind == 0) {
     switch (cfg) {
-      case 0: launch_grouped_cfg<128, 64, 4, 1, 2, false>(t, n, grid, s, tc); break;
-      case 1: launch_grouped_cfg<128, 128, 2, 2, 2, false>(t, n, grid, s, tc); break;
-      case 2: launch_grouped_cfg<64, 128, 2, 2, 2, false>(t, n, grid, s, tc); break;
-      default: launch_grouped_cfg<64, 64, 2, 2, 3, false>(t, n, grid, s, tc); break;
+      case 0: launch_grouped_cfg<128, 64, 4, 1, 2, false>(t, n, grid, s, tc, r2); break;
+      case 1: launch_grouped_cfg<128, 128, 2, 2, 2, false>(t, n, grid, s, tc, r2); break;
+      case 2: launch_grouped_cfg<64, 128, 2, 2, 2, false>(t, n, grid, s, tc, r2); break;
+      default: launch_grouped_cfg<64, 64, 2, 2, 3, false>(t, n, grid, s, tc, r2); break;
     }
   } else {
     switch (cfg) {
-      case 0: launch_grouped_cfg<128, 64, 4, 1, 2, true>(t, n, grid, s, tc); break;
-      case 1: launch_grouped_cfg<128, 128, 2, 2, 2, true>(t, n, grid, s, tc); break;
-      case 2: launch_grouped_cfg<64, 128, 2, 2, 2, true>(t, n, grid, s, tc); break;
-      default: launch_grouped_cfg<64, 64, 2, 2, 3, true>(t, n, grid, s, tc); break;
+      case 0: launch_grouped_cfg<128, 64, 4, 1, 2, true>(t, n, grid, s, tc, r2); break;
+      case 1: launch_grouped_cfg<128, 128, 2, 2, 2, true>(t, n, grid, s, tc, r2); break;
+      case 2: launch_grouped_cfg<64, 128, 2, 2, 2, true>(t, n, grid, s, tc, r2); break;
+      default: launch_grouped_cfg<64, 64, 2, 2, 3, true>(t, n, grid, s, tc, r2); break;
     }
   }
   if (route_probe_on()) return MXDET_OK;
diff --git a/mxdetection_amd/models/backbones/resnet.py b/mxdetection_amd/models/backbones/resnet.py
--- a/mxdetection_amd/models/backbones/resnet.py
+++ b/mxdetection_amd/models/backbones/resnet.py
@@ -92,8 +92,17 @@
     def backward(self, ds, dx_buf, dx_has_grad):
         c1, c2, c3 = self.conv1, self.conv2, self.conv3
         c3.backward_weight(self.a2, ds)
-        d_a2 = c3.backward_data(ds, self.a2.shape, relu_mask=self.a2, out=self._buf("d_a2", self.a2.shape),
-                                relu_bits=self.a2_bits)
+        d_a2 = self._buf("d_a2", self.a2.shape)
+        dsc = None
+        if self.down is not None and self.need_dx:
+            assert self.down.stride == 2
+            dsc = self._buf("dsc", ds.shape[:3] + (self.down.cin,))
+            kw = {} if self.a2_bits is None else dict(relu_bits=self.a2_bits)
+            dense.conv2d_group("dgrad", [c3.dgrad_call(ds, self.a2.shape, relu_mask=self.a2, out=d_a2, **kw),
+                                         self.down.compact_dgrad_call(ds, dx_buf if dx_has_grad else None, out=dsc)],
+                               c1.device)
+        else:
+            c3.backward_data(ds, self.a2.shape, relu_mask=self.a2, out=d_a2, relu_bits=self.a2_bits)
         c2.backward_weight(self.a1, d_a2)
         d_a1 = c2.backward_data(d_a2, self.a1.shape, relu_mask=self.a1, out=self._buf("d_a1", self.a1.shape),
                                 relu_bits=self.a1_bits)
@@ -104,8 +113,8 @@
             return None
         xb = self.x_bits
         if self.down is not None:
-            self.down.backward_data(ds, self.x.shape, accumulate=dx_has_grad, out=dx_buf)
-            c1.backward_data(d_a1, self.x.shape, residual=dx_buf, relu_mask=self.x, out=dx_buf, relu_bits=xb)
+            c1.backward_data(d_a1, self.x.shape, residual=dx_buf if dx_has_grad else None, relu_mask=self.x, out=dx_buf,
+                             relu_bits=xb, res_sub=dsc)
         else:
             if dx_has_grad:
                 dense.add_bf16(dx_buf, ds, dx_buf)
diff --git a/mxdetection_amd/models/utils/layers.py b/mxdetection_amd/models/utils/layers.py
--- a/mxdetection_amd/models/utils/layers.py
+++ b/mxdetection_amd/models/utils/layers.py
@@ -179,12 +179,19 @@
         t = (dy, self.wt, tuple(x_shape), self.k, self.k, self.stride, self.pad, residual, relu_mask, accumulate, out)
         return t if relu_bits is None else t + (relu_bits,)
 
-    def backward_data(self, dy, x_shape, residual=None, relu_mask=None, accumulate=False, out=None, relu_bits=None):
+    def compact_dgrad_call(self, dy, lateral=None, out=None):
+        assert self.k == 1 and self.pad == 0 and self.stride > 1
+        N, Ho, Wo, _ = dy.shape
+        return (dy, self.wt, (N, Ho, Wo, self.cin), 1, 1, 1, 0, lateral, None, False, out, None, None,
+                self.stride if lateral is not None else None)
+
+    def backward_data(self, dy, x_shape, residual=None, relu_mask=None, accumulate=False, out=None, relu_bits=None,
+                      res_sub=None):
         if dense.PF_TRACE is not None:
             dense.PF_TRACE.append((self, "b", dense.mem_range(self.wt), None))
         return dense.conv2d_dgrad(dy, self.wt, x_shape, self.k, self.k, self.stride, self.pad, residual,
                                   None if relu_bits is not None else relu_mask, accumulate, out, prefetch=self.pf_bwd,
-                                  relu_bits=relu_bits)
+                                  relu_bits=relu_bits, res_sub=res_sub)
 
     def backward_weight(self, x, dy, accumulate=False):
         if self.ws.grouping and not accumulate:
diff --git a/mxdetection_amd/ops/dense.py b/mxdetection_amd/ops/dense.py
--- a/mxdetection_amd/ops/dense.py
+++ b/mxdetection_amd/ops/dense.py
@@ -20,8 +20,14 @@
 
 
 def conv_desc(N, H, W, Cin, Cout, KH, KW, stride, pad, relu=False, res_upsample=False, accumulate=False, prefetch=None,
-              relu_bits=None):
+              relu_bits=None, res_sub=None, res_strided=None):
     d = ConvDescT()
+    if res_sub is not None:
+        if tuple(res_sub.shape) != (N, (H + 1) // 2, (W + 1) // 2, Cin) or res_sub.dtype != torch.bfloat16:
+            raise ValueError("res_sub %s does not match a [%d,%d,%d,%d] data gradient" % (tuple(res_sub.shape), N, H, W, Cin))
+        d.res_sub = res_sub.data_ptr()
+    if res_strided is not None:
+        d.res_stride, d.res_h, d.res_w = res_strided
     if relu_bits is not None:
         d.relu_bits = relu_bits.data_ptr()
     if prefetch is not None:
@@ -77,13 +83,25 @@
     return out if w3 is None else (out, out3)
 
 
+def _strided_residual(residual, res_stride, x_shape):
+    if res_stride is None or res_stride <= 1:
+        return None
+    N, H, W, Cin = x_shape
+    if (residual is None or residual.shape[0] != N or residual.shape[3] != Cin or
+            residual.shape[1] < (H - 1) * res_stride + 1 or residual.shape[2] < (W - 1) * res_stride + 1):
+        raise ValueError("a residual read with pixel stride %d must cover the [%d,%d,%d,%d] data gradient" %
+                         (res_stride, N, H, W, Cin))
+    return (res_stride, residual.shape[1], residual.shape[2])
+
+
 def conv2d_dgrad(dy, wt, x_shape, KH, KW, stride=1, pad=0, residual=None, relu_mask=None, accumulate=False, out=None,
-                 prefetch=None, relu_bits=None):
+                 prefetch=None, relu_bits=None, res_sub=None, res_stride=None):
     lib = _lib.load()
     N, H, W, Cin = x_shape
     Cout = dy.shape[3]
     d = conv_desc(N, H, W, Cin, Cout, KH, KW, stride, pad, relu=(relu_mask is not None or relu_bits is not None),
-                  accumulate=accumulate, prefetch=prefetch, relu_bits=relu_bits)
+                  accumulate=accumulate, prefetch=prefetch, relu_bits=relu_bits, res_sub=res_sub,
+                  res_strided=_strided_residual(residual, res_stride, x_shape))
     if out is None:
         out = torch.empty(tuple(x_shape), dtype=torch.bfloat16, device=dy.device)
     check(lib.mxdet_conv2d_dgrad(C.byref(d), ptr(dy), ptr(wt), ptr(residual), ptr(relu_mask), ptr(out), stream_ptr()),
@@ -137,7 +155,8 @@
                 N, H, W, Cin = x_shape
                 Cout = dy.shape[3]
                 it.desc = conv_desc(N, H, W, Cin, Cout, KH, KW, stride, pad, relu=(relu_mask is not None or bits is not None),
-                                    accumulate=accumulate, prefetch=hint, relu_bits=bits)
+                                    accumulate=accumulate, prefetch=hint, relu_bits=bits, res_sub=c[12] if len(c) > 12 else None,
+                                    res_strided=_strided_residual(residual, c[13] if len(c) > 13 else None, x_shape))
                 hint = None
                 it.src, it.filt, it.bias, it.residual, it.relu_mask, it.dst = (dp(dy), dp(wt), None, dp(residual),
                                                                               None if bits is not None else dp(relu_mask), dp(out))
@@ -183,7 +202,8 @@
         else:
             dy, wt, x_shape, KH, KW, stride, pad, residual, relu_mask, accumulate, out = c[:11]
             conv2d_dgrad(dy, wt, x_shape, KH, KW, stride, pad, residual, relu_mask, accumulate, out,
-                         relu_bits=c[11] if len(c) > 11 else None)
+                         relu_bits=c[11] if len(c) > 11 else None, res_sub=c[12] if len(c) > 12 else None,
+                         res_stride=c[13] if len(c) > 13 else None)
 
 
 class GroupedWgrad:
```

Measured after the change: 450.3 images/sec. No clear change (-0.1%).
